# idiap/ilqr_planner

Hardware: AMD Instinct MI355X
Metric: iLQR iterations/sec (7-DoF, T=200, batch 4096) + final-cost rel-err vs Eigen ref (higher is better)
Workload: dtype f64; 1 GPU; C3: PosOrn nb_deriv=1 7-DoF Panda chain, T=200, batch 4096/GPU x 1 GPU = 4096, solver=al, 20 iterations/solve, line search on, early stop off; global_batch=4096, horizon=200, parallelism=instances sharded x1, exchange=none

## Files before the change

### ilqr_planner_amd/capi.py

```python
from __future__ import annotations

import collections
import ctypes as C
import os

import numpy as np

_HERE = os.path.dirname(os.path.abspath(__file__))
LIB_PATH = os.path.join(_HERE, "libilqr_hip.so")

MAX_SEG, MAX_KP, MAX_NX, MAX_NU, MAX_NF, MAX_NQ = 24, 8, 15, 8, 15, 13
SYS_POS_ORN, SYS_POS_ORN_TIME, SYS_JOINT, SYS_JOINT_TIME = 0, 1, 2, 3
STATUS_OK, STATUS_NONFINITE, STATUS_ALPHA_FLOOR, STATUS_SWEEP_IO = 0, 1, 2, 4
LQT_MAX_NX, LQT_MAX_NU = 16, 8
CL_STATS = 5
KP_ERR, KP_STATS, CL_OUTCOME = 5, 12, 4
CL_CON_STATS, CL_OUTCOME_CON = 6, 5
KP_ERR_POS, KP_ERR_ORN, KP_ERR_VEL, KP_ERR_ANGVEL, KP_ERR_TIME = range(5)
PROF_ROLLOUT, PROF_BACKWARD, PROF_FORWARD, PROF_OTHER, PROF_APPLY = 0, 1, 2, 3, 4
ADOPT_STATE, ADOPT_TARGETS, ADOPT_CONTROLS0, ADOPT_CONTROLS, ADOPT_MULTIPLIERS = 1, 2, 4, 8, 16
CLR_MAX_SPH, CLR_MAX_PLANES, CLR_STATS = 32, 8, 4

EXPORTS = [
    "ilqr_dims_of", "ilqr_desc_defaults", "ilqr_ctx_create", "ilqr_ctx_destroy", "ilqr_last_error", "ilqr_ctx_set_stream",
# ... 230 lines not shown
    L.ilqr_problem_closed_loop_dev.argtypes = [vp, C.c_int, vp, vp, C.c_int, vp, vp, vp]
    L.ilqr_problem_closed_loop_noise.argtypes = [vp, C.c_int, C.POINTER(Noise), dp, C.c_int, dp, dp, dp, dp, dp]
    L.ilqr_problem_closed_loop_noise_dev.argtypes = [vp, C.c_int, C.POINTER(Noise), vp, C.c_int, vp, vp, vp, vp, vp]
    L.ilqr_problem_closed_loop_report.argtypes = [vp, C.c_int, C.POINTER(Noise), dp, dp, C.c_int, C.POINTER(Tol), dp, dp, C.POINTER(Report)]
    L.ilqr_problem_closed_loop_report_dev.argtypes = [vp, C.c_int, C.POINTER(Noise), vp, vp, C.c_int, C.POINTER(Tol), vp, vp, C.POINTER(Report)]
    L.ilqr_problem_closed_loop_cov.argtypes = [vp, dp, dp, C.POINTER(Cov)]
    L.ilqr_problem_closed_loop_cov_dev.argtypes = [vp, dp, dp, C.POINTER(Cov)]
    L.ilqr_problem_closed_loop_report_con.argtypes = [vp, C.c_int, C.POINTER(Noise), dp, dp, C.c_int, C.POINTER(Tol), dp, dp, C.POINTER(Report),
                                                      C.c_double, C.POINTER(Con)]
    L.ilqr_problem_closed_loop_report_con_dev.argtypes = [vp, C.c_int, C.POINTER(Noise), vp, vp, C.c_int, C.POINTER(Tol), vp, vp, C.POINTER(Report),
                                                          C.c_double, C.POINTER(Con)]
    L.ilqr_problem_closed_loop_cov_con.argtypes = [vp, dp, dp, C.POINTER(Cov), C.POINTER(CovCon)]
    L.ilqr_problem_closed_loop_cov_con_dev.argtypes = [vp, dp, dp, C.POINTER(Cov), C.POINTER(CovCon)]
    L.ilqr_solve_recursive.argtypes = [vp, C.c_int, C.c_int, C.c_int]
    L.ilqr_solve_al.argtypes = [vp, C.c_int, C.c_int, C.c_double, C.c_double, C.c_int, C.c_int]
    L.ilqr_solve_batch_cp.argtypes = [vp, dp, C.c_int, C.c_int, C.c_int]
    L.ilqr_solve_batch.argtypes = [vp, C.c_int, C.c_int]
    for n in ("X", "fX", "U", "K", "d", "cost", "alpha", "lambda", "X_dev", "U_dev", "cost_dev"):
        getattr(L, "ilqr_problem_get_" + n).argtypes = [vp, vp]
    L.ilqr_problem_get_iters.argtypes = [vp, ip]
    L.ilqr_problem_get_status.argtypes = [vp, ip]
    L.ilqr_problem_get_trace.argtypes = [vp, dp, dp, C.c_int]
    L.ilqr_fk_batch.argtypes = [vp, C.POINTER(ProblemDesc), C.c_int, dp, dp, dp, dp]
    L.ilqr_profile_enable.argtypes = [vp, C.c_int]
    L.ilqr_profile_reset.argtypes = [vp]
    L.ilqr_profile_get.argtypes = [vp, C.c_int, dp, ip]
    L.ilqr_chain_from_urdf.argtypes = [C.c_char_p, C.c_char_p, C.c_char_p, dp, dp, C.POINTER(ProblemDesc), dp, dp]
    L.ilqr_urdf_last_error.restype = C.c_char_p
    _lib = L
    return L


def _dp(a):
    return a.ctypes.data_as(C.POINTER(C.c_double)) if a is not None else None


def _f64(x, shape=None):
    a = np.ascontiguousarray(np.asarray(x, dtype=np.float64))
    if shape is not None and tuple(a.shape) != tuple(shape):
        raise ValueError(f"expected shape {tuple(shape)}, got {a.shape}")
    return a


def _out(want, *shape):
    return np.empty(shape) if want else None


def chain_from_urdf(urdf_text: str, base: str, tip: str, tool_rpy=None, tool_xyz=None):
    L = load()
    d = ProblemDesc()
    L.ilqr_desc_defaults(C.byref(d))
    lo, up = np.zeros(MAX_SEG), np.zeros(MAX_SEG)
    rpy = _f64(tool_rpy, (3,)) if tool_rpy is not None else None
    xyz = _f64(tool_xyz, (3,)) if tool_xyz is not None else None
    if L.ilqr_chain_from_urdf(urdf_text.encode(), base.encode(), tip.encode(), _dp(rpy), _dp(xyz), C.byref(d), _dp(lo), _dp(up)):
        raise RuntimeError(L.ilqr_urdf_last_error().decode())
    n = d.n_seg
    return dict(dof=d.dof, seg_joint=[d.seg_joint[i] for i in range(n)], seg_xyz=[list(d.seg_xyz[i]) for i in range(n)],
                seg_R=[list(d.seg_R[i]) for i in range(n)], seg_axis=[list(d.seg_axis[i]) for i in range(n)],
                lower=lo[: d.dof].copy(), upper=up[: d.dof].copy())


def make_desc(*, kind, nb_deriv, horizon, dt, R_diag, chain, kp_timesteps, kp_Q, limits=None, kp_dist=None, kp_frames=None, kp_Ru=None,
              limit_multiplicity=1, kp_joint=None, limits2=None) -> ProblemDesc:
    L = load()
    d = ProblemDesc()
    L.ilqr_desc_defaults(C.byref(d))
    d.kind, d.nb_deriv, d.dof, d.horizon, d.dt = int(kind), int(nb_deriv), int(chain["dof"]), int(horizon), float(dt or 0.0)
    for i, v in enumerate(R_diag):
        d.R_diag[i] = float(v)
    n = len(chain["seg_joint"])
    if n > MAX_SEG:
        raise ValueError("too many segments")
    d.n_seg = n
    for i in range(n):
        d.seg_joint[i] = int(chain["seg_joint"][i])
        for k in range(3):
            d.seg_xyz[i][k] = float(chain["seg_xyz"][i][k])
            d.seg_axis[i][k] = float(chain["seg_axis"][i][k])
        for k in range(9):
            d.seg_R[i][k] = float(chain["seg_R"][i][k])
    dims = Dims()
    if L.ilqr_dims_of(C.byref(d), C.byref(dims)):
        raise ValueError("unsupported system kind / nb_deriv")
    if limits is not None:
        d.limits_set, d.penalty = 1, float(limits.get("penalty", 1.0))
        for i in range(len(limits["state_max"])):
            d.state_max[i] = float(limits["state_max"][i])
            d.state_min[i] = float(limits["state_min"][i])
            d.limit_weight[i] = int(limits["limit_weight"][i])
    d.n_kp = len(kp_timesteps)
    nq = dims.n_Q
    for k, (ts, Q) in enumerate(zip(kp_timesteps, kp_Q)):
        d.kp_timestep[k] = int(ts)
        jk = bool(kp_joint and kp_joint[k])
        d.kp_joint[k] = int(jk)
        nqk = dims.n_x if jk else nq
        Q = _f64(Q, (nqk, nqk))
        for a in range(nqk):
            for b in range(nqk):
                d.kp_Q[k][a * nqk + b] = Q[a, b]
    d.limit_multiplicity = int(limit_multiplicity)
    if limits2 is not None:
        d.is_sequence, d.limits2_set, d.penalty2 = 1, 1, float(limits2.get("penalty", 1.0))
        d.limit_multiplicity2 = int(limits2.get("multiplicity", 1))
        for i in range(len(limits2["state_max"])):
            d.state_max2[i] = float(limits2["state_max"][i])
            d.state_min2[i] = float(limits2["state_min"][i])
            d.limit_weight2[i] = int(limits2["limit_weight"][i])
    for k, fr in enumerate(kp_frames or []):
        if fr is not None:
            Tm = _f64(fr, (4, 4))
            d.kp_has_frame[k] = 1
            for a in range(3):
                d.kp_frame_p[k][a] = Tm[a, 3]
                for b in range(3):
                    d.kp_frame_R[k][a * 3 + b] = Tm[a, b]
    for k, ru in enumerate(kp_Ru or []):
        if ru is not None:
            d.kp_has_Ru[k] = 1
            for a, v in enumerate(ru):
                d.kp_Ru[k][a] = float(v)
    for k, kd in enumerate(kp_dist or []):
        if kd is not None:
            d.kp_dist[k] = 1
            d.kp_pos_radius[k] = float(kd["pos_radius"])
            for i in range(3):
                d.kp_orn_thresh[k][i] = float(kd["orn_thresh"][i])
    return d


class Context:
    def __init__(self, device_id: int = 0):
        import weakref

        self.L = load()
        self.h = C.c_void_p()
        self._problems = weakref.WeakSet()
        self.obstacle_path = 0
        rc = self.L.ilqr_ctx_create(device_id, C.byref(self.h))
        if rc:
            raise RuntimeError(f"ilqr_ctx_create failed (code {rc}): no usable HIP device {device_id}; there is no CPU fallback")

    def check(self, rc):
        if rc:
            raise RuntimeError(self.L.ilqr_last_error(self.h).decode())

    def set_stream(self, stream_ptr):
        self.check(self.L.ilqr_ctx_set_stream(self.h, C.c_void_p(stream_ptr)))

    def synchronize(self):
        self.check(self.L.ilqr_ctx_synchronize(self.h))

    _PINS = {"sweep": {None: 0, "mfma": 1, "rows": 2, "siwave": 4, "siwg": 5, "siwgio": 6, "siwgprep": 7}, "forward": {None: 0, "wg": 1, "dpp": 2, "wglds": 3}, "reroll": {None: 0, "rows": 1, "dpp": 2}}

    def set_crosscheck(self, generic_kernels=False, cp_lane_solve=False, cp_general=False, sweep=None, forward=None, reroll=None):
        pins = []
        for name, v in (("sweep", sweep), ("forward", forward), ("reroll", reroll)):
            if v not in self._PINS[name]:
                raise ValueError(f"set_crosscheck: {name} must be one of {[k for k in self._PINS[name] if k]} or None (got {v!r})")
            pins.append(self._PINS[name][v])
        self.check(self.L.ilqr_ctx_set_crosscheck(self.h, int(bool(generic_kernels)), int(bool(cp_lane_solve)), int(bool(cp_general)), *pins))

    def crosscheck_from_env(self):
        env = os.environ
        self.set_crosscheck(env.get("ILQR_HIP_PATH") == "v1", env.get("ILQR_CP_SOLVE") == "lane", env.get("ILQR_CP") == "general",
                            sweep=env.get("ILQR_SWEEP") or None, forward=env.get("ILQR_FWD") or None, reroll=env.get("ILQR_APPLY") or None)

    OBSTACLE_PATHS = {"generic": 0, "cooperative": 1}

    def set_obstacle_path(self, path):
        if isinstance(path, str):
            if path not in self.OBSTACLE_PATHS:
                raise ValueError(f"set_obstacle_path: path must be one of {list(self.OBSTACLE_PATHS)} (got {path!r})")
            path = self.OBSTACLE_PATHS[path]
        self.check(self.L.ilqr_ctx_set_obstacle_path(self.h, int(path)))
        self.obstacle_path = int(path)

    def set_split(self, mode: int):
        self.check(self.L.ilqr_ctx_set_split(self.h, int(mode)))

    def profile(self, on: bool):
        self.check(self.L.ilqr_profile_enable(self.h, int(on)))

    def profile_reset(self):
        self.check(self.L.ilqr_profile_reset(self.h))

    def profile_get(self, which):
        ms, n = C.c_double(), C.c_int()
        self.check(self.L.ilqr_profile_get(self.h, which, C.byref(ms), C.byref(n)))
        return ms.value, n.value

    def fk_batch(self, desc: ProblemDesc, q):
        q = _f64(q)
        n, dof = q.shape
        pos, quat, jac = np.zeros((n, 3)), np.zeros((n, 4)), np.zeros((n, 6, dof))
        self.check(self.L.ilqr_fk_batch(self.h, C.byref(desc), n, _dp(q), _dp(pos), _dp(quat), _dp(jac)))
        return pos, quat, jac

    def clearance_trajectories(self, desc: ProblemDesc, X, robot: ClrRobot, obstacles=None, traj_per_set=None, margin: float = 0.0, stats_group=None,
                               want=CLR_OUTPUTS):
        X = _f64(X)
        n, T = X.shape[0], X.shape[1]
        want = tuple(want) + (("stats",) if stats_group is not None else ())
        return _clr_host_call(lambda r, w, o: self.check(self.L.ilqr_clearance_trajectories(self.h, C.byref(desc), n, T, X.ctypes.data, r, w, o)),
                              n, T, robot, obstacles, n if traj_per_set is None else traj_per_set, margin, stats_group, want)

    def clearance_trajectories_dev(self, desc: ProblemDesc, n: int, T: int, X_ptr, robot: ClrRobot, world: ClrWorld, out: ClrOut):
        self.check(self.L.ilqr_clearance_trajectories_dev(self.h, C.byref(desc), int(n), int(T), X_ptr, C.byref(robot), C.byref(world), C.byref(out)))

    def close(self):
        if self.h:
            for p in list(self._problems):
                p.close()
            self.L.ilqr_ctx_destroy(self.h)
            self.h = C.c_void_p()

    def __del__(self):
        try:
            self.close()
        except Exception:
            pass


class BatchProblem:

    def __init__(self, ctx: Context, desc: ProblemDesc, batch: int):
        self.ctx, self.L, self.desc, self.B = ctx, ctx.L, desc, int(batch)
        self.dims = Dims()
        self.L.ilqr_dims_of(C.byref(desc), C.byref(self.dims))
        self.T, self.n_kp = desc.horizon, int(desc.n_kp)
        self.h = C.c_void_p()
        ctx.check(self.L.ilqr_problem_create(ctx.h, C.byref(desc), self.B, C.byref(self.h)))
        ctx._problems.add(self)
        self.m = 0

    def set_init_state(self, q0, dq0=None):
        q0 = _f64(q0, (self.B, self.desc.dof))
        dq0 = _f64(dq0, (self.B, self.desc.dof)) if dq0 is not None else None
        self.ctx.check(self.L.ilqr_problem_set_init_state(self.h, q0.ctypes.data, dq0.ctypes.data if dq0 is not None else None))

    def set_keypoint_targets(self, k, target):
        t = _f64(target, (self.B, self.dims.n_f))
        self.ctx.check(self.L.ilqr_problem_set_keypoint_targets(self.h, k, t.ctypes.data))

    def set_controls(self, U0):
        U0 = _f64(U0, (self.B, self.T - 1, self.dims.n_u))
        self.ctx.check(self.L.ilqr_problem_set_controls(self.h, U0.ctypes.data))

    def set_constraints(self, A, b, lambda0=None):
        A, b = _f64(A), _f64(b)
        per_step = 1 if A.ndim == 3 else 0
        self.m = A.shape[-2]
        lam = _f64(lambda0, (self.B, self.T - 1, self.m)) if lambda0 is not None else None
        self.ctx.check(self.L.ilqr_problem_set_constraints(self.h, self.m, per_step, _dp(A), _dp(b), _dp(lam)))

    def reset_multipliers(self):
        self.ctx.check(self.L.ilqr_problem_reset_multipliers(self.h))

    def set_init_state_dev(self, q0_ptr, dq0_ptr=None):
        self.ctx.check(self.L.ilqr_problem_set_init_state_dev(self.h, q0_ptr, dq0_ptr))

    def set_keypoint_targets_dev(self, k, ptr):
        self.ctx.check(self.L.ilqr_problem_set_keypoint_targets_dev(self.h, k, ptr))

    def set_controls_dev(self, ptr):
        self.ctx.check(self.L.ilqr_problem_set_controls_dev(self.h, ptr))

    def solve_recursive(self, nb_iter, line_search=True, early_stop=True):
        self.ctx.crosscheck_from_env()
        self.ctx.check(self.L.ilqr_solve_recursive(self.h, nb_iter, int(line_search), int(early_stop)))

    def solve_al(self, nb_iter, lag_update_step, penalty, scaling_factor, line_search=True, early_stop=True):
        self.ctx.crosscheck_from_env()
        self.ctx.check(self.L.ilqr_solve_al(self.h, nb_iter, lag_update_step, penalty, scaling_factor, int(line_search), int(early_stop)))

    def solve_batch_cp(self, psi, nb_iter, early_stop=True):
        psi = _f64(psi)
        assert psi.shape[0] == (self.T - 1) * self.dims.n_u
        self.ctx.crosscheck_from_env()
        self.ctx.check(self.L.ilqr_solve_batch_cp(self.h, _dp(psi), psi.shape[1], nb_iter, int(early_stop)))

    def solve_batch(self, nb_iter, early_stop=True):
        self.ctx.check(self.L.ilqr_solve_batch(self.h, nb_iter, int(early_stop)))

    def _get(self, name, shape):
        o = np.zeros(shape)
        self.ctx.check(getattr(self.L, "ilqr_problem_get_" + name)(self.h, o.ctypes.data))
        return o

    def X(self):
        return self._get("X", (self.B, self.T, self.dims.n_x))

    def fX(self):
        return self._get("fX", (self.B, self.T, self.dims.n_f))

    def U(self):
        return self._get("U", (self.B, self.T - 1, self.dims.n_u))

    def K(self):
        return self._get("K", (self.B, self.T - 1, self.dims.n_u, self.dims.n_x))

    def d(self):
        return self._get("d", (self.B, self.T - 1, self.dims.n_u))

    def cost(self):
        return self._get("cost", (self.B,))
# ... 405 lines not shown
```

### ilqr_planner_amd/csrc/ilqr_capi.cpp

```cpp
#include "../../include/ilqr_hip.h"

#include <hip/hip_runtime.h>

#include <cmath>
#include <cstdio>
#include <cstdlib>
#include <cstring>
#include <string>
#include <vector>

#include "ilqr_batchcp.hpp"
#include "ilqr_clearance.hpp"
#include "ilqr_closed_loop.hpp"
#include "ilqr_closed_loop_cov.hpp"
#include "ilqr_ctx.hpp"
#include "ilqr_kernels.hpp"
#include "ilqr_multistart.hpp"
#include "ilqr_obstacle.hpp"
#include "ilqr_plan.hpp"

using namespace ilqr;

struct DevScratch {
    double* ptr = nullptr;
    size_t elems = 0;
    int reserve(ilqr_ctx* c, size_t n) {
        if (elems >= n) return 0;
        if (ptr) { HIPCHK(c, hipStreamSynchronize(c->stream)); HIPCHK(c, hipFree(ptr)); ptr = nullptr; elems = 0; }
        HIPCHK(c, hipMalloc((void**)&ptr, n * sizeof(double)));
        elems = n;
        return 0;
    }
    void release() { if (ptr) (void)hipFree(ptr); ptr = nullptr; elems = 0; }
};

struct ilqr_problem {
    ilqr_ctx* ctx = nullptr;
    ilqr_problem_desc desc;
    ilqr_dims udims;
    ilqr_dims dims;
    DofMap map;
    bool mapped = false;
    IndexMap qmap;
    int B = 0, Bp = 0, T = 0;
    DevDesc hdesc;
    DevDesc* ddesc = nullptr;
    DevDesc* ddesc_half[2] = {nullptr, nullptr};
    int half_b0[2] = {0, 0}, half_B[2] = {0, 0};
    Bufs bufs;
    std::vector<void*> allocs;
    double *conA = nullptr, *conb = nullptr;
    double* lambda0 = nullptr;
    bool con_state_only = false;
    int trace_iters = 0;
    DevScratch staging;
    int last_nb_iter = 0;
    bool has_controls = false, has_state = false;
    bool has_gains = false;
    bool has_plan = false;
    DevScratch cl_cost;
    DevScratch cl_kpx;
    DevScratch cl_rep;
    DevScratch cl_con_ws;
    DevScratch cl_cov_ws;
    DevScratch cl_cov_kps;
    DevScratch ms_idx;
    DevScratch ms_out;
    bool has_obs = false;
    ObsArgs obs = {};
    size_t obs_sets_bytes = 0;
    ObsDense obs_dense = {};
    bool u0_zero = false;
    BatchCPState cp;
    BatchWideState cpw;
};


extern "C" const char* ilqr_version(void) { return "ilqr_hip 0.1 (gfx950, fp64)"; }

extern "C" void ilqr_desc_defaults(ilqr_problem_desc* d) {
    std::memset(d, 0, sizeof(*d));
    d->reg = 1e-6;
    d->alpha_floor = 1e-3;
    d->stop_tol = 1e-3;
    d->nb_deriv = 1;
    d->dof = 7;
}

extern "C" int ilqr_dims_of(const ilqr_problem_desc* d, ilqr_dims* o) {
    if (!d || !o) return 1;
    if (d->kind != ILQR_SYS_POS_ORN && d->kind != ILQR_SYS_POS_ORN_TIME && d->kind != ILQR_SYS_JOINT && d->kind != ILQR_SYS_JOINT_TIME) return 1;
    if (d->nb_deriv != 1 && d->nb_deriv != 2) return 1;
    if (d->kind == ILQR_SYS_JOINT || d->kind == ILQR_SYS_JOINT_TIME) {
        if (d->nb_deriv != 1) return 1;
        o->n_x = o->n_u = o->n_f = o->n_Q = d->dof + (d->kind == ILQR_SYS_JOINT_TIME ? 1 : 0);
        return 0;
    }
    const int tm = d->kind == ILQR_SYS_POS_ORN_TIME ? 1 : 0;
    o->n_x = d->nb_deriv * d->dof + tm;
    o->n_u = d->dof + tm;
    o->n_f = 7 * d->nb_deriv + tm;
    o->n_Q = o->n_f - d->nb_deriv;
    return 0;
}

extern "C" int ilqr_ctx_create(int device_id, ilqr_ctx** out) {
    if (!out) return 1;
    *out = nullptr;
    int n = 0;
    if (hipGetDeviceCount(&n) != hipSuccess || n <= 0) return 2;
    if (device_id < 0 || device_id >= n) return 3;
    if (hipSetDevice(device_id) != hipSuccess) return 4;
    auto* c = new ilqr_ctx();
    c->device = device_id;
    if (hipStreamCreateWithFlags(&c->own_stream, hipStreamNonBlocking) != hipSuccess) {
        delete c;
        return 5;
    }
    c->stream = c->own_stream;
    { int cus = 0; if (hipDeviceGetAttribute(&cus, hipDeviceAttributeMultiprocessorCount, device_id) == hipSuccess && cus > 0) c->n_simd = 4 * cus; }
    *out = c;
    return 0;
}

static void clr_release(ilqr_ctx* c);

extern "C" void ilqr_ctx_destroy(ilqr_ctx* c) {
    if (!c) return;
    (void)hipSetDevice(c->device);
    while (!c->problems.empty()) ilqr_problem_destroy(c->problems.back());
    while (!c->cleanups.empty()) { const auto cl = c->cleanups.back(); cl.destroy(cl.handle); }
    (void)hipStreamSynchronize(c->stream);
    clr_release(c);
    for (auto& p : c->pending) (void)hipEventDestroy(p.a);
    for (auto e : c->pool) (void)hipEventDestroy(e);
    for (int i = 0; i < 2; i++) {
        if (c->half_stream[i]) (void)hipStreamSynchronize(c->half_stream[i]);
        if (c->half_stream[i]) (void)hipStreamDestroy(c->half_stream[i]);
        if (c->ev_half_done[i]) (void)hipEventDestroy(c->ev_half_done[i]);
    }
    if (c->ev_begin) (void)hipEventDestroy(c->ev_begin);
    if (c->ev_stagger) (void)hipEventDestroy(c->ev_stagger);
    if (c->own_stream) (void)hipStreamDestroy(c->own_stream);
    delete c;
}

extern "C" const char* ilqr_last_error(const ilqr_ctx* c) { return c ? c->err.c_str() : "null context"; }

extern "C" int ilqr_ctx_set_stream(ilqr_ctx* c, void* s) {
    if (!c) return 1;
    c->stream = s ? (hipStream_t)s : c->own_stream;
    return 0;
}

extern "C" int ilqr_ctx_set_split(ilqr_ctx* c, int on) {
    if (!c) return 1;
    if (on < 0 || on > 2) return fail(c, "ilqr_ctx_set_split: mode must be 0, 1 or 2 (got " + std::to_string(on) + ")");
    c->split = on;
    return 0;
}

static_assert((int)SweepPin::Mfma == ILQR_XC_SWEEP_MFMA && (int)SweepPin::Rows == ILQR_XC_SWEEP_ROWS && (int)SweepPin::SiWave == ILQR_XC_SWEEP_SI_WAVE &&
              (int)SweepPin::SiWg == ILQR_XC_SWEEP_SI_WG && (int)SweepPin::SiWgIo == ILQR_XC_SWEEP_SI_WG_IO && (int)SweepPin::SiWgPrep == ILQR_XC_SWEEP_SI_WG_PREP && (int)FwdPin::Wg == ILQR_XC_FWD_WG &&
              (int)FwdPin::Dpp == ILQR_XC_FWD_DPP && (int)FwdPin::WgLds == ILQR_XC_FWD_WG_LDS && (int)RerollPin::Rows == ILQR_XC_REROLL_ROWS && (int)RerollPin::Dpp == ILQR_XC_REROLL_DPP,
              "variant pins of ilqr_plan.hpp and include/ilqr_hip.h");

extern "C" int ilqr_ctx_set_crosscheck(ilqr_ctx* c, int generic_kernels, int cp_lane_solve, int cp_general, int sweep, int forward, int reroll) {
    if (!c) return 1;
    if (sweep < 0 || sweep > 7 || sweep == 3) return fail(c, "ilqr_ctx_set_crosscheck: sweep must be ILQR_XC_AUTO, ILQR_XC_SWEEP_MFMA, ILQR_XC_SWEEP_ROWS, ILQR_XC_SWEEP_SI_WAVE, ILQR_XC_SWEEP_SI_WG, ILQR_XC_SWEEP_SI_WG_IO or ILQR_XC_SWEEP_SI_WG_PREP");
    if (forward < 0 || forward > 3) return fail(c, "ilqr_ctx_set_crosscheck: forward must be ILQR_XC_AUTO, ILQR_XC_FWD_WG, ILQR_XC_FWD_DPP or ILQR_XC_FWD_WG_LDS");
    if (reroll < 0 || reroll > 2) return fail(c, "ilqr_ctx_set_crosscheck: reroll must be ILQR_XC_AUTO, ILQR_XC_REROLL_ROWS or ILQR_XC_REROLL_DPP");
    c->xc_sweep = (SweepPin)sweep;
    c->xc_forward = (FwdPin)forward;
    c->xc_reroll = (RerollPin)reroll;
    c->xc_generic = generic_kernels != 0;
    c->xc_cp_lane = cp_lane_solve != 0;
    c->xc_cp_general = cp_general != 0;
    return 0;
}

extern "C" int ilqr_ctx_set_obstacle_path(ilqr_ctx* c, int path) {
    if (!c) return 1;
    if (path != ILQR_OBSTACLE_PATH_GENERIC && path != ILQR_OBSTACLE_PATH_COOPERATIVE)
        return fail(c, "ilqr_ctx_set_obstacle_path: path must be ILQR_OBSTACLE_PATH_GENERIC (0) or ILQR_OBSTACLE_PATH_COOPERATIVE (1) (got " + std::to_string(path) + ")");
    c->obs_coop = path == ILQR_OBSTACLE_PATH_COOPERATIVE;
    return 0;
}

extern "C" int ilqr_ctx_synchronize(ilqr_ctx* c) {
    if (!c) return 1;
    HIPCHK(c, hipStreamSynchronize(c->stream));
    return 0;
}


static hipEvent_t ev_get(ilqr_ctx* c) {
    if (!c->pool.empty()) {
        hipEvent_t e = c->pool.back();
        c->pool.pop_back();
        return e;
    }
    hipEvent_t e;
    (void)hipEventCreate(&e);
    return e;
}
static void prof_collect(ilqr_ctx* c) {
    if (c->pending.empty()) return;
    (void)hipStreamSynchronize(c->stream);
    for (size_t i = 0; i + 1 < c->pending.size(); i++) {
        const auto& p = c->pending[i];
        float ms = 0;
        if (p.which >= 0 && hipEventElapsedTime(&ms, p.a, c->pending[i + 1].a) == hipSuccess) {
            c->prof_ms[p.which] += ms;
            c->prof_n[p.which] += 1;
        }
    }
    for (auto& p : c->pending) c->pool.push_back(p.a);
    c->pending.clear();
}
static void prof_mark(ilqr_ctx* c, int which) {
    if (!c->profile) return;
    hipEvent_t e = ev_get(c);
    (void)hipEventRecord(e, c->stream);
    c->pending.push_back({e, nullptr, which});
    if (which < 0 && c->pending.size() > 4096) prof_collect(c);
}
struct ProfScope {
    ProfScope(ilqr_ctx* c, int w) { prof_mark(c, w); }
};

static void prof_hook_fn(void* c, int which) { prof_mark((ilqr_ctx*)c, which); }
static ilqr::ProfHook prof_hook(ilqr_ctx* c) {
    ilqr::ProfHook h;
    if (c->profile) { h.mark = prof_hook_fn; h.ctx = c; }
    return h;
}

extern "C" int ilqr_profile_enable(ilqr_ctx* c, int on) {
    if (!c) return 1;
    prof_collect(c);
    c->profile = on != 0;
    return 0;
}
extern "C" int ilqr_profile_reset(ilqr_ctx* c) {
    if (!c) return 1;
    prof_collect(c);
    for (int i = 0; i < ILQR_PROF_COUNT; i++) { c->prof_ms[i] = 0; c->prof_n[i] = 0; }
    return 0;
}
extern "C" int ilqr_profile_get(ilqr_ctx* c, int which, double* ms, int* n) {
    if (!c || which < 0 || which >= ILQR_PROF_COUNT) return 1;
    prof_collect(c);
    if (ms) *ms = c->prof_ms[which];
    if (n) *n = c->prof_n[which];
    return 0;
}


static void mat3(const double* A, const double* B, double* C) {
    for (int i = 0; i < 3; i++)
        for (int j = 0; j < 3; j++) C[3 * i + j] = A[3 * i] * B[j] + A[3 * i + 1] * B[3 + j] + A[3 * i + 2] * B[6 + j];
}

static_assert(DOF == DEV_DOF, "ilqr_dofmap.hpp and ilqr_device.hpp");
static_assert(STEP_MAX_KP == ILQR_MAX_KP && MAX_KP == ILQR_MAX_KP, "ilqr_steps.hpp, ilqr_device.hpp and include/ilqr_hip.h");

static int check_dof(ilqr_ctx* c, int dof) {
    if (dof < 1 || dof > DOF) return fail(c, "chains of 1 to 7 moving joints are supported (dof = " + std::to_string(dof) + ")");
    return 0;
}

static int lower_chain(ilqr_ctx* c, const ilqr_problem_desc& d, DevChain& ch) {
    if (check_dof(c, d.dof)) return 1;
    if (d.n_seg < 1 || d.n_seg > ILQR_MAX_SEG) return fail(c, "bad n_seg");
    double R[9] = {1, 0, 0, 0, 1, 0, 0, 0, 1}, p[3] = {0, 0, 0};
    int nj = 0;
    for (int s = 0; s < d.n_seg; s++) {
        double Rn[9];
        for (int i = 0; i < 3; i++) p[i] += R[3 * i] * d.seg_xyz[s][0] + R[3 * i + 1] * d.seg_xyz[s][1] + R[3 * i + 2] * d.seg_xyz[s][2];
        mat3(R, d.seg_R[s], Rn);
        std::memcpy(R, Rn, sizeof(R));
        const int j = d.seg_joint[s];
        if (j >= 0) {
            if (j != nj) return fail(c, "moving joints must be numbered 0..dof-1 in chain order");
            if (nj >= DOF) return fail(c, "chain has more than 7 moving joints (chains of 1 to 7 moving joints are supported)");
            std::memcpy(ch.Rpre[nj], R, sizeof(R));
            std::memcpy(ch.ppre[nj], p, sizeof(p));
            std::memcpy(ch.axis[nj], d.seg_axis[s], 3 * sizeof(double));
            nj++;
            const double I[9] = {1, 0, 0, 0, 1, 0, 0, 0, 1};
            std::memcpy(R, I, sizeof(R));
            p[0] = p[1] = p[2] = 0;
        }
    }
    if (nj != d.dof)
        return fail(c, "chain has " + std::to_string(nj) + " moving joints, descriptor says " + std::to_string(d.dof) + " (chains of 1 to 7 moving joints are supported)");
    for (int j = nj; j < DOF; j++) {
        const double I[9] = {1, 0, 0, 0, 1, 0, 0, 0, 1};
        std::memcpy(ch.Rpre[j], I, sizeof(I));
        for (int i = 0; i < 3; i++) ch.ppre[j][i] = ch.axis[j][i] = 0.0;
    }
    std::memcpy(ch.Rtail, R, sizeof(R));
    std::memcpy(ch.ptail, p, sizeof(p));
    return 0;
}

static int lower_desc(ilqr_ctx* c, const ilqr_problem_desc& d, const DofMap& m, int B, int Bp, DevDesc& h) {
    ilqr_dims dm;
    if (ilqr_dims_of(&d, &dm)) return fail(c, "unsupported system kind / nb_deriv");
    const IndexMap &mx = m.x, &mu = m.u;
    auto xs = [&](const double* v, int j) { return mx.usr[j] < 0 ? 0.0 : v[mx.usr[j]]; };
    auto xi = [&](const int* v, int j) { return mx.usr[j] < 0 ? 0 : v[mx.usr[j]]; };
    auto us = [&](const double* v, int j) { return v[mu.usr[j] < 0 ? 0 : mu.usr[j]]; };
    std::memset(&h, 0, sizeof(h));
    if (!((d.kind == ILQR_SYS_JOINT || d.kind == ILQR_SYS_JOINT_TIME) && d.n_seg == 0) && lower_chain(c, d, h.chain)) return 1;
    if (d.horizon < 2) return fail(c, "horizon must be >= 2");
    h.kind = d.kind; h.nd = d.nb_deriv; h.T = d.horizon; h.B = B; h.Bp = Bp; h.dt = d.dt;
    for (int j = 0; j < mu.n_dev; j++) h.R_diag[j] = us(d.R_diag, j);
    {
        const double mult = d.limit_multiplicity > 1 ? (double)d.limit_multiplicity : 1.0;
        h.limits_set = d.limits_set;
        h.penalty = d.penalty * mult;
        h.pen_xx = d.penalty * d.penalty * mult;
// ... 212 lines not shown
extern "C" int ilqr_problem_set_controls_dev(ilqr_problem* p, const double* U0) { return set_controls(p, U0, true); }

extern "C" int ilqr_problem_set_constraints(ilqr_problem* p, int m, int per_step, const double* A, const double* b, const double* lambda0) {
    if (!p) return 1;
    ilqr_ctx* c = p->ctx;
    if (m <= 0 || !A || !b) return fail(c, "bad constraint arguments");
    p->has_gains = p->has_plan = false;
    const int ns = p->dims.n_x + p->dims.n_u, T = p->T, nsu = p->udims.n_x + p->udims.n_u;
    const size_t nk = per_step ? (size_t)(T - 1) : 1;
    if (p->bufs.m != m || p->bufs.per_step != per_step || !p->conA) {
        if (p->conA) {
            HIPCHK(c, hipStreamSynchronize(c->stream));
            void* old[5] = {p->conA, p->conb, p->bufs.lambda, p->bufs.Is, p->lambda0};
            for (void* q : old) {
                for (auto it = p->allocs.begin(); it != p->allocs.end(); ++it)
                    if (*it == q) { p->allocs.erase(it); break; }
                (void)hipFree(q);
            }
            p->conA = p->conb = p->lambda0 = nullptr;
            p->bufs.lambda = p->bufs.Is = nullptr;
            p->bufs.m = 0;
        }
        if (dalloc(p, &p->conA, nk * m * ns) || dalloc(p, &p->conb, nk * m)) return 1;
        double *lam, *Is;
        if (dalloc(p, &lam, (size_t)(T - 1) * m * p->Bp) || dalloc(p, &Is, (size_t)(T - 1) * m * p->Bp)) return 1;
        p->bufs.lambda = lam;
        p->bufs.Is = Is;
        if (dalloc(p, &p->lambda0, (size_t)(T - 1) * m * p->Bp)) return 1;
    }
    std::vector<double> Aw;
    if (p->mapped) {
        const IndexMap &mx = p->map.x, &mu = p->map.u;
        Aw.assign(nk * m * ns, 0.0);
        for (size_t r = 0; r < nk * m; r++) {
            for (int j = 0; j < mx.n_user; j++) Aw[r * ns + mx.dev[j]] = A[r * nsu + j];
            for (int i = 0; i < mu.n_user; i++) Aw[r * ns + mx.n_dev + mu.dev[i]] = A[r * nsu + mx.n_user + i];
        }
    }
    HIPCHK(c, hipMemcpyAsync(p->conA, p->mapped ? Aw.data() : A, nk * m * ns * sizeof(double), hipMemcpyHostToDevice, c->stream));
    HIPCHK(c, hipMemcpyAsync(p->conb, b, nk * m * sizeof(double), hipMemcpyHostToDevice, c->stream));
    HIPCHK(c, hipStreamSynchronize(c->stream));
    p->bufs.m = m; p->bufs.per_step = per_step; p->bufs.conA = p->conA; p->bufs.conb = p->conb;
    p->con_state_only = true;
    for (size_t k = 0; k < nk * m; k++)
        for (int j = p->udims.n_x; j < nsu; j++)
            if (A[k * nsu + j] != 0.0) p->con_state_only = false;
    if (lambda0) {
        if (upload(p, lambda0, false, p->bufs.lambda, (T - 1) * m)) return 1;
    } else {
        HIPCHK(c, hipMemsetAsync(p->bufs.lambda, 0, sizeof(double) * (size_t)(T - 1) * m * p->Bp, c->stream));
    }
    HIPCHK(c, hipMemcpyAsync(p->lambda0, p->bufs.lambda, sizeof(double) * (size_t)(T - 1) * m * p->Bp, hipMemcpyDeviceToDevice, c->stream));
    return 0;
}

extern "C" int ilqr_problem_reset_multipliers(ilqr_problem* p) {
    if (!p) return 1;
    if (p->bufs.m <= 0) return fail(p->ctx, "no constraints set");
    p->has_gains = p->has_plan = false;
    HIPCHK(p->ctx, hipMemcpyAsync(p->bufs.lambda, p->lambda0, sizeof(double) * (size_t)(p->T - 1) * p->bufs.m * p->Bp,
                                  hipMemcpyDeviceToDevice, p->ctx->stream));
    return 0;
}


static int ensure_trace(ilqr_problem* p, int nb_iter) {
    if (nb_iter > p->trace_iters) {
        double *ct, *at;
        if (dalloc(p, &ct, (size_t)nb_iter * p->Bp, false) || dalloc(p, &at, (size_t)nb_iter * p->Bp, false)) return 1;
        p->bufs.cost_trace = ct;
        p->bufs.alpha_trace = at;
        p->trace_iters = nb_iter;
    }
    if (nb_iter > 0) {
        HIPCHK(p->ctx, hipMemsetAsync(p->bufs.cost_trace, 0xFF, sizeof(double) * (size_t)nb_iter * p->Bp, p->ctx->stream));
        HIPCHK(p->ctx, hipMemsetAsync(p->bufs.alpha_trace, 0xFF, sizeof(double) * (size_t)nb_iter * p->Bp, p->ctx->stream));
    }
    return 0;
}

static Bufs half_bufs(const ilqr_problem* p, int half) {
    Bufs v = p->bufs;
    const size_t o = (size_t)p->half_b0[half];
    v.desc = p->ddesc_half[half];
    for (int i = 0; i < 2; i++) { v.X[i] += o; v.U[i] += o; }
    v.U0 += o; v.q0 += o; v.dq0 += o; v.kp_tg += o;
    v.KD += o * (size_t)kd_rs(p->bufs.kd_sym, p->dims.n_u, kd_rowp(p->dims.n_x));
    v.cost += o; v.alpha += o; v.cur += o; v.active += o; v.iters += o; v.status += o; v.kpd += o; v.pend += o; v.pred += o;
    v.lsc += o; v.dun += o; v.kpdev += o; v.kpx += o; v.dunA += o;
    if (v.ws) v.ws += o;
    if (v.cost_trace) { v.cost_trace += o; v.alpha_trace += o; }
    if (v.lambda) { v.lambda += o; v.Is += o; }
    return v;
}

static PlanIn plan_input(const ilqr_problem* p, bool al, int nb_iter, int line_search) {
    const ilqr_ctx* c = p->ctx;
    const int T = p->T;
    PlanIn in;
    in.kind = p->desc.kind; in.nd = p->desc.nb_deriv; in.al = al; in.m = p->bufs.m; in.per_step = p->bufs.per_step; in.con_state_only = p->con_state_only;
    in.limits2_set = p->desc.limits2_set != 0;
    in.shared_steps = has_shared_step(p->hdesc.steps);
    in.obstacles = p->has_obs;
    in.obstacles_coop = c->obs_coop;
    in.uniform_R = true;
    for (int i = 1; i < p->dims.n_u; i++) in.uniform_R = in.uniform_R && (p->hdesc.R_diag[i] == p->hdesc.R_diag[0]);
    in.off32 = (size_t)2 * T * p->dims.n_x * p->Bp * 8 < ((size_t)1 << 32) && (size_t)T * (p->bufs.m > 0 ? p->bufs.m : 1) * p->Bp * 8 < ((size_t)1 << 32);
    in.line_search = line_search != 0; in.alpha_floor = p->desc.alpha_floor; in.nb_iter = nb_iter;
    in.B = p->B; in.n_simd = c->n_simd; in.halves = p->ddesc_half[0] != nullptr; in.split = c->split; in.profile = c->profile;
    in.generic = c->xc_generic; in.sweep = c->xc_sweep; in.forward = c->xc_forward; in.reroll = c->xc_reroll;
    return in;
}

struct Half { Bufs bufs; int B; hipStream_t st; };
static int split_begin(ilqr_problem* p, bool split, Half hv[2], int& nh) {
    ilqr_ctx* c = p->ctx;
    nh = 1;
    if (!split) {
        hv[0].bufs = p->bufs; hv[0].B = p->B; hv[0].st = c->stream;
        return 0;
    }
    for (int i = 0; i < 2; i++) {
        if (!c->half_stream[i]) HIPCHK(c, hipStreamCreateWithFlags(&c->half_stream[i], hipStreamNonBlocking));
        if (!c->ev_half_done[i]) HIPCHK(c, hipEventCreateWithFlags(&c->ev_half_done[i], hipEventDisableTiming));
    }
    if (!c->ev_begin) HIPCHK(c, hipEventCreateWithFlags(&c->ev_begin, hipEventDisableTiming));
    if (!c->ev_stagger) HIPCHK(c, hipEventCreateWithFlags(&c->ev_stagger, hipEventDisableTiming));
    HIPCHK(c, hipEventRecord(c->ev_begin, c->stream));
    nh = 2;
    for (int i = 0; i < 2; i++) {
        HIPCHK(c, hipStreamWaitEvent(c->half_stream[i], c->ev_begin, 0));
        hv[i].bufs = half_bufs(p, i); hv[i].B = p->half_B[i]; hv[i].st = c->half_stream[i];
    }
    return 0;
}
struct SplitJoin {
    ilqr_ctx* c; bool on;
    ~SplitJoin() {
        if (!on) return;
        for (int i = 0; i < 2; i++)
            if (hipEventRecord(c->ev_half_done[i], c->half_stream[i]) != hipSuccess || hipStreamWaitEvent(c->stream, c->ev_half_done[i], 0) != hipSuccess)
                (void)hipStreamSynchronize(c->half_stream[i]);
    }
};

static FwdArgs plan_fwd_args(const ilqr_problem* p, const RiccatiPlan& pl) {
    FwdArgs f;
    std::memset(&f, 0, sizeof(f));
    f.n_alpha = pl.n_alpha; f.n_kp = p->hdesc.steps.n;
    f.shared = has_shared_step(p->hdesc.steps) ? 1 : 0;
    f.n_kp_all = p->desc.n_kp;
    f.fused = pl.fused ? 1 : 0;
    f.fwd_lds = pl.fwd_lds ? 1 : 0;
    f.limits = p->desc.limits_set ? 1 : 0;
    for (int k = 0; k < p->desc.n_kp; k++) f.kp_ext |= p->desc.kp_dist[k] | p->desc.kp_has_frame[k] | p->desc.kp_has_Ru[k] | p->desc.kp_joint[k];
    return f;
}
static void launch_sweep(const ilqr_problem* p, const RiccatiPlan& pl, int h, bool al, const Bufs& bf, int B, hipStream_t st, SweepArgs& sw) {
    const int kind = p->desc.kind, nd = p->desc.nb_deriv;
    switch (pl.sweep) {
        case Sweep::SiDpp: sw.si_wg = pl.si_wg[h] ? 1 : 0; sw.si_io = pl.si_io[h] ? 1 : 0; sw.si_prep = pl.si_prep[h] ? 1 : 0; launch_backward_si_dpp(al, pl.fused, pl.kd_sym == 1, pl.si_lanes[h], bf, B, st, sw); break;
        case Sweep::Rows: launch_backward_rows(kind, nd, al, bf, B, st); break;
        case Sweep::Mfma: launch_backward_mfma(kind, nd, al, bf, B, st); break;
        case Sweep::Generic: launch_backward_generic(kind, nd, al, bf, B, st, p->has_obs ? &p->obs : nullptr); break;
    }
}
static void launch_obs_terms(const ilqr_problem* p, const RiccatiPlan& pl, const Bufs& bf, int B, hipStream_t st) {
    if (!p->has_obs) return;
    launch_obs_derivs(bf, p->obs, B, p->T, p->dims.n_x, 0, st);
    if (pl.obs_dense) launch_stage_dense(bf, p->obs, p->obs_dense.sd, B, p->T, 0, st);
}
static int ensure_obs_dense(ilqr_problem* p) {
    ilqr_ctx* c = p->ctx;
    const int N = p->dims.n_x;
    if (!p->obs_dense.sd) HIPCHK(c, hipMalloc((void**)&p->obs_dense.sd, sizeof(double) * (size_t)p->T * (size_t)(N + N * N) * (size_t)p->Bp));
    if (!p->obs_dense.part) HIPCHK(c, hipMalloc((void**)&p->obs_dense.part, sizeof(double) * (size_t)p->T * OBS_LS_ROWS * (size_t)p->Bp));
    return 0;
}

static int solve_riccati(ilqr_problem* p, bool al, int nb_iter, int lag, double penalty0, double scaling, int line_search, int early_stop) {
    if (!p) return 1;
    ilqr_ctx* c = p->ctx;
    if (!p->has_state || !p->has_controls) return fail(c, "set_init_state and set_controls must be called before a solve");
    if (nb_iter < 0) return fail(c, "nb_iter < 0");
    if (al && (p->bufs.m <= 0 || lag <= 0)) return fail(c, "AL solve needs constraints (ilqr_problem_set_constraints) and lag_update_step > 0");
    HIPCHK(c, hipSetDevice(c->device));
    if (ensure_trace(p, nb_iter)) return 1;
    p->last_nb_iter = nb_iter;
    p->has_gains = p->has_plan = false;
    const int kind = p->desc.kind, nd = p->desc.nb_deriv, T = p->T;
    const RiccatiPlan pl = plan_riccati(plan_input(p, al, nb_iter, line_search));
    if (pl.kd_sym != KD_SYM_KEEP) p->bufs.kd_sym = pl.kd_sym;
    if (pl.needs_ws && !p->bufs.ws)
        if (dalloc(p, &p->bufs.ws, (size_t)backward_ws_entries(kind, nd) * p->Bp, false)) return 1;
    if (pl.obs_dense && ensure_obs_dense(p)) return 1;

    Half hv[2];
    int nh = 1;
    if (split_begin(p, pl.split, hv, nh)) return 1;
    SplitJoin split_join{c, pl.split};
    FwdArgs f = plan_fwd_args(p, pl);
    f.line_search = line_search; f.early_stop = early_stop; f.nb_iter = nb_iter; f.penalty_roll = penalty0; f.al = al ? 1 : 0;
    if (pl.obs_dense) { f.obs = &p->obs; f.obs_part = p->obs_dense.part; f.obs_T = T; }
    for (int h = 0; h < nh; h++) {
        const Bufs& bf = hv[h].bufs;
        ProfScope ps(c, ILQR_PROF_ROLLOUT);
        if (pl.init == Init::Lti) launch_init_lti(kind, nd, bf, hv[h].B, hv[h].st);
        else launch_init(kind, nd, al, bf, hv[h].B, hv[h].st, penalty0, p->has_obs ? &p->obs : nullptr);
        if (pl.obs_dense) launch_obs_ls(bf, p->obs, p->obs_dense.part, hv[h].B, T, p->dims.n_x, 1, 1, hv[h].st);
        if (pl.init_al_update) {
            f.it = -1; f.do_update = 0;
            launch_al_update(kind, nd, bf, hv[h].B, T, hv[h].st, f);
        }
    }
    HIPCHK(c, hipGetLastError());
    double penalty = penalty0;
    SweepArgs sw;
    sw.pen_in = penalty; sw.pen_update_prev = penalty; sw.do_update_prev = 0; sw.si_wg = 0; sw.si_io = 0; sw.si_prep = 0;
    sw.sd = pl.obs_dense ? p->obs_dense.sd : nullptr;
    for (int it = 0; it < nb_iter; it++) {
        FwdArgs fi = f;
        fi.it = it;
        fi.penalty_roll = penalty;
        fi.do_update = al && ((it + 1) % lag == 0);
        if (fi.do_update) penalty *= scaling;
        fi.penalty_update = penalty;
        for (int h = 0; h < nh; h++) {
            const Bufs& bf = hv[h].bufs;
            const int B = hv[h].B;
            hipStream_t st = hv[h].st;
            if (pl.split && it == 0 && h == 1) HIPCHK(c, hipStreamWaitEvent(st, c->ev_stagger, 0));
            {
                ProfScope ps(c, ILQR_PROF_OTHER);
                launch_kp_derivs(kind, nd, bf, B, st, fi);
                launch_obs_terms(p, pl, bf, B, st);
            }
            {
                ProfScope ps(c, ILQR_PROF_BACKWARD);
                launch_sweep(p, pl, h, al, bf, B, st, sw);
            }
            if (pl.split && it == 0 && h == 0) HIPCHK(c, hipEventRecord(c->ev_stagger, st));
            {
                ProfScope ps(c, ILQR_PROF_FORWARD);
                switch (pl.forward) {
                    case Forward::WaveWg: launch_forward_wave(kind, false, bf, B, st, fi); break;
                    case Forward::WaveDpp: launch_forward_wave(kind, true, bf, B, st, fi); break;
                    case Forward::Lin: launch_forward_lin(bf, B, st, fi); break;
                    case Forward::Mfma: launch_forward_tm(kind, nd, bf, B, st, fi); break;
                    case Forward::Generic: launch_forward_generic(kind, nd, al, bf, B, st, fi, p->has_obs ? &p->obs : nullptr); break;
                }
            }
            if (pl.apply != Apply::None && (pl.apply != Apply::WaveLast || it == nb_iter - 1)) {
                ProfScope ps(c, ILQR_PROF_APPLY);
                switch (pl.apply) {
                    case Apply::Wave: case Apply::WaveLast: launch_apply_wave(kind, bf, B, T, st, fi); break;
                    case Apply::Lin: launch_apply_lin(bf, B, T, st); break;
                    case Apply::RerollRows: case Apply::RerollDpp: launch_apply_tm(kind, nd, pl.apply == Apply::RerollDpp, bf, B, st, fi); break;
                    case Apply::None: break;
                }
            }
            if (pl.al_update) {
                ProfScope ps(c, ILQR_PROF_OTHER);
                launch_al_update(kind, nd, bf, B, T, st, fi);
            }
        }
        sw.pen_in = fi.penalty_roll; sw.pen_update_prev = fi.penalty_update; sw.do_update_prev = fi.do_update;
        HIPCHK(c, hipGetLastError());
    }
    prof_mark(c, -1);
    p->has_gains = nb_iter >= 1;
    p->has_plan = true;
    return 0;
}

extern "C" int ilqr_solve_recursive(ilqr_problem* p, int nb_iter, int line_search, int early_stop) {
    return solve_riccati(p, false, nb_iter, 1, 0.0, 1.0, line_search, early_stop);
}
extern "C" int ilqr_solve_al(ilqr_problem* p, int nb_iter, int lag, double penalty, double scaling, int line_search, int early_stop) {
    return solve_riccati(p, true, nb_iter, lag, penalty, scaling, line_search, early_stop);
}

static const char* const BATCH_SHARED_STEP_TEXT =
    "keypoints that share a timestep are not supported by the batch solvers (ilqr_solve_batch_cp, ilqr_solve_batch)";
static const char* const BATCH_OBSTACLES_TEXT =
    "obstacle terms are not supported by the batch solvers (ilqr_solve_batch_cp, ilqr_solve_batch): remove them (ilqr_problem_set_obstacles with robot = NULL) or use ilqr_solve_recursive / ilqr_solve_al";

extern "C" int ilqr_solve_batch_cp(ilqr_problem* p, const double* psi, int Kw, int nb_iter, int early_stop) {
    if (!p) return 1;
    ilqr_ctx* c = p->ctx;
    if (has_shared_step(p->hdesc.steps)) return fail(c, BATCH_SHARED_STEP_TEXT);
    if (p->has_obs) return fail(c, BATCH_OBSTACLES_TEXT);
    if (!p->has_state || !p->has_controls) return fail(c, "set_init_state and set_controls must be called before a solve");
    p->has_gains = p->has_plan = false;
    HIPCHK(c, hipSetDevice(c->device));
    std::string err;
    if (ensure_trace(p, nb_iter)) return 1;
    p->last_nb_iter = nb_iter;
    const bool cp_time = p->desc.kind == ILQR_SYS_POS_ORN_TIME || p->desc.kind == ILQR_SYS_JOINT_TIME;
    std::vector<double> psiw;
    if (psi && Kw > 0 && p->mapped) {
        const IndexMap& mu = p->map.u;
        psiw.assign((size_t)(p->T - 1) * mu.n_dev * Kw, 0.0);
        for (int k = 0; k < p->T - 1; k++)
            for (int i = 0; i < mu.n_user; i++)
                std::memcpy(&psiw[((size_t)k * mu.n_dev + mu.dev[i]) * Kw], psi + ((size_t)k * mu.n_user + i) * Kw, sizeof(double) * Kw);
        psi = psiw.data();
// ... 1121 lines not shown
```

### ilqr_planner_amd/csrc/ilqr_kernels.hpp

```cpp
#pragma once
#include <hip/hip_runtime.h>

#include "ilqr_device.hpp"
#include "ilqr_dofmap.hpp"

namespace ilqr {

struct ObsArgs;

struct Bufs {
    const DevDesc* desc;
    double* X[2];
    double* U[2];
    const double* U0;
    double* KD;
    const double* q0;
    const double* dq0;
    const double* kp_tg;
    double* cost;
    double* alpha;
    int* cur;
    int* active;
    int* iters;
    int* status;
    double* kpd;
    int* pend;
    int* pred;
    double* lsc;
    double* dun;
    double* kpdev;
    double* kpx;
    double* dunA;
    double* ws;
    double* cost_trace;
    double* alpha_trace;
    int m, per_step;
    const double* conA;
    const double* conb;
    double* lambda;
    double* Is;
    int kd_sym;
};

constexpr int kd_rowp(int nx) { return (nx + 2) & ~1; }
constexpr int KD_SYM_RS = 36, KD_SYM_D = 28;
__host__ __device__ constexpr int kd_sym_tri(int i, int j) { return i * 7 - i * (i - 1) / 2 + (j - i); }
__host__ __device__ constexpr int kd_sym_off(int i, int j) { return j >= 7 ? KD_SYM_D + i : (i <= j ? kd_sym_tri(i, j) : kd_sym_tri(j, i)); }
__host__ __device__ inline int kd_off(int sym, int rowp, int i, int j) { return sym ? kd_sym_off(i, j) : i * rowp + j; }
__host__ __device__ inline int kd_rs(int sym, int nu, int rowp) { return sym ? KD_SYM_RS : nu * rowp; }
#define KD_REC(kd, Bp, RS, k, b) ((kd) + ((size_t)(k) * (size_t)(Bp) + (size_t)(b)) * (size_t)(RS))

struct FwdArgs {
    int it, line_search, early_stop, do_update, nb_iter;
    int n_kp;
    int shared;
    int n_kp_all;
    int al;
    int n_alpha;
    double penalty_roll, penalty_update;
    int kp_ext;
    int limits;
    int fused;
    int fwd_lds;
    const ObsArgs* obs;
    double* obs_part;
    int obs_T;
};

struct SweepArgs {
    double pen_in;
    double pen_update_prev;
    int do_update_prev;
    int si_wg;
    int si_io;
    int si_prep;
    const double* sd;
};

void launch_init(int kind, int nd, bool al, const Bufs& a, int B, hipStream_t st, double penalty, const ObsArgs* o = nullptr);
void launch_gains_prepare(const Bufs& a, int B, hipStream_t st);
void launch_gains_al_weights(int kind, int nd, const Bufs& a, int B, int T, double penalty, hipStream_t st);
void launch_kp_derivs(int kind, int nd, const Bufs& a, int B, hipStream_t st, const FwdArgs& f);
void launch_backward_generic(int kind, int nd, bool al, const Bufs& a, int B, hipStream_t st, const ObsArgs* o = nullptr);
int backward_ws_entries(int kind, int nd);
void launch_forward_generic(int kind, int nd, bool al, const Bufs& a, int B, hipStream_t st, const FwdArgs& f, const ObsArgs* o = nullptr);
void launch_init_lti(int kind, int nd, const Bufs& a, int B, hipStream_t st);
void launch_backward_si_dpp(bool al, bool fused, bool uniform_R, int lpi, const Bufs& a, int B, hipStream_t st, const SweepArgs& sw);
void launch_backward_rows(int kind, int nd, bool al, const Bufs& a, int B, hipStream_t st);
void launch_backward_mfma(int kind, int nd, bool al, const Bufs& a, int B, hipStream_t st);
void launch_forward_wave(int kind, bool small, const Bufs& a, int B, hipStream_t st, const FwdArgs& f);
void launch_apply_wave(int kind, const Bufs& a, int B, int T, hipStream_t st, const FwdArgs& f);
void launch_forward_lin(const Bufs& a, int B, hipStream_t st, const FwdArgs& f);
void launch_apply_lin(const Bufs& a, int B, int T, hipStream_t st);
void launch_forward_tm(int kind, int nd, const Bufs& a, int B, hipStream_t st, const FwdArgs& f);
void launch_apply_tm(int kind, int nd, bool dpp, const Bufs& a, int B, hipStream_t st, const FwdArgs& f);
void launch_al_update(int kind, int nd, const Bufs& a, int B, int T, hipStream_t st, const FwdArgs& f);
void launch_fx_all(int kind, int nd, const Bufs& a, int B, int T, double* out, hipStream_t st);
void launch_to_soa(const double* src, double* dst, int B, int Bp, int rows, hipStream_t st);
void launch_from_soa(const double* src, double* dst, int B, int Bp, int rows, hipStream_t st);
void launch_from_soa_cur(const double* s0, const double* s1, const int* cur, double* dst, int B, int Bp, int rows, hipStream_t st);
void launch_from_soa_scaled(const double* src, const double* alpha, const int* iters, double* dst, int B, int Bp, int rows, hipStream_t st);
void launch_get_gains(const double* kd, int kd_sym, const double* alpha, const int* iters, double* K_out, double* d_out, int B, int Bp, int T1, int nu, int nx, hipStream_t st);
void launch_warm_start(const Bufs& a, double* U0, double* q0, double* dq0, int shift, int B, int T, int nx, int nu, int nd, hipStream_t st);
void launch_track(const Bufs& a, const double* x_meas, int k, int with_ff, double* u_out, int B, int nx, int nu, hipStream_t st);
void launch_closed_loop_stats(const double* cost, int B, int S, double* stats, hipStream_t st);
void launch_fk_batch(const DevDesc* dd, int n, const double* q, double* pos, double* quat, double* jac, hipStream_t st);
void launch_to_soa_map(const double* src, double* dst, int B, int Bp, int outer, const IndexMap& m, hipStream_t st);
void launch_from_soa_cur_map(const double* s0, const double* s1, const int* cur, double* dst, int B, int Bp, int outer, const IndexMap& m,
                             hipStream_t st);
void launch_get_gains_map(const double* kd, int kd_sym, const double* alpha, const int* iters, double* K_out, double* d_out, int B, int Bp, int T1,
                          const DofMap& m, hipStream_t st);
void launch_track_map(const Bufs& a, const double* x_meas, int k, int with_ff, double* u_out, int B, const DofMap& m, hipStream_t st);

}
```

### ilqr_planner_amd/csrc/ilqr_kernels_dpp.hip

```cpp
#include "../../include/ilqr_hip.h"
#include "ilqr_kernels.hpp"
#include "ilqr_lanes.hpp"
#include "ilqr_step.hpp"

namespace ilqr {

namespace {

#define DPPM_ALL " row_mask:0xf bank_mask:0xf"
#define DPPM_LO " row_mask:0xf bank_mask:0x3"
#define DPPM_HI " row_mask:0xf bank_mask:0xc"


template <int LPI>
__device__ __forceinline__ void fmac_rows_all(double (&acc)[7], const double (&src)[7], const double (&mul)[7]) {
#define R_(K, LL, MASK)                                                                                                                   \
    "v_fmac_f64_dpp %[a0], %[s0], %[m" #K "] row_newbcast:" LL MASK "\n\tv_fmac_f64_dpp %[a1], %[s1], %[m" #K "] row_newbcast:" LL MASK "\n\t" \
    "v_fmac_f64_dpp %[a2], %[s2], %[m" #K "] row_newbcast:" LL MASK "\n\tv_fmac_f64_dpp %[a3], %[s3], %[m" #K "] row_newbcast:" LL MASK "\n\t" \
    "v_fmac_f64_dpp %[a4], %[s4], %[m" #K "] row_newbcast:" LL MASK "\n\tv_fmac_f64_dpp %[a5], %[s5], %[m" #K "] row_newbcast:" LL MASK "\n\t" \
    "v_fmac_f64_dpp %[a6], %[s6], %[m" #K "] row_newbcast:" LL MASK "\n\t"
#define OPS_                                                                                                                              \
    : [a0] "+v"(acc[0]), [a1] "+v"(acc[1]), [a2] "+v"(acc[2]), [a3] "+v"(acc[3]), [a4] "+v"(acc[4]), [a5] "+v"(acc[5]), [a6] "+v"(acc[6])    \
    : [s0] "v"(src[0]), [s1] "v"(src[1]), [s2] "v"(src[2]), [s3] "v"(src[3]), [s4] "v"(src[4]), [s5] "v"(src[5]), [s6] "v"(src[6]),          \
      [m0] "v"(mul[0]), [m1] "v"(mul[1]), [m2] "v"(mul[2]), [m3] "v"(mul[3]), [m4] "v"(mul[4]), [m5] "v"(mul[5]), [m6] "v"(mul[6])
    if (LPI == 16)
        asm volatile("s_nop 1\n\t" R_(0, "0", DPPM_ALL) R_(1, "1", DPPM_ALL) R_(2, "2", DPPM_ALL) R_(3, "3", DPPM_ALL) R_(4, "4", DPPM_ALL) R_(5, "5", DPPM_ALL)
                         R_(6, "6", DPPM_ALL) "s_nop 0" OPS_);
    else
        asm volatile("s_nop 1\n\t" R_(0, "0", DPPM_LO) R_(0, "8", DPPM_HI) R_(1, "1", DPPM_LO) R_(1, "9", DPPM_HI) R_(2, "2", DPPM_LO) R_(2, "10", DPPM_HI)
                         R_(3, "3", DPPM_LO) R_(3, "11", DPPM_HI) R_(4, "4", DPPM_LO) R_(4, "12", DPPM_HI) R_(5, "5", DPPM_LO) R_(5, "13", DPPM_HI)
                             R_(6, "6", DPPM_LO) R_(6, "14", DPPM_HI) "s_nop 0" OPS_);
#undef R_
#undef OPS_
}
template <int LPI>
__device__ __forceinline__ double row_dot_bc(const double (&M)[7], double src) {
    double s0, s1, s2;
#define D_(A, K, LL, MASK) "v_fmac_f64_dpp %[" A "], %[x], %[m" #K "] row_newbcast:" LL MASK "\n\t"
#define OPS_                                                                                                                       \
    : [s0] "=&v"(s0), [s1] "=&v"(s1), [s2] "=&v"(s2)                                                                                \
    : [x] "v"(src), [m0] "v"(M[0]), [m1] "v"(M[1]), [m2] "v"(M[2]), [m3] "v"(M[3]), [m4] "v"(M[4]), [m5] "v"(M[5]), [m6] "v"(M[6])
#define ZERO_ "v_mov_b64 %[s0], 0\n\tv_mov_b64 %[s1], 0\n\tv_mov_b64 %[s2], 0\n\ts_nop 1\n\t"
    if (LPI == 16)
        asm volatile(ZERO_ D_("s0", 0, "0", DPPM_ALL) D_("s1", 1, "1", DPPM_ALL) D_("s2", 2, "2", DPPM_ALL) D_("s0", 3, "3", DPPM_ALL) D_("s1", 4, "4", DPPM_ALL)
                         D_("s2", 5, "5", DPPM_ALL) D_("s0", 6, "6", DPPM_ALL) "s_nop 0" OPS_);
    else
        asm volatile(ZERO_ D_("s0", 0, "0", DPPM_LO) D_("s1", 1, "1", DPPM_LO) D_("s2", 2, "2", DPPM_LO) D_("s0", 0, "8", DPPM_HI) D_("s1", 1, "9", DPPM_HI)
                         D_("s2", 2, "10", DPPM_HI) D_("s0", 3, "3", DPPM_LO) D_("s1", 4, "4", DPPM_LO) D_("s2", 5, "5", DPPM_LO) D_("s0", 3, "11", DPPM_HI)
                             D_("s1", 4, "12", DPPM_HI) D_("s2", 5, "13", DPPM_HI) D_("s0", 6, "6", DPPM_LO) "s_nop 1\n\t" D_("s0", 6, "14", DPPM_HI) "s_nop 0" OPS_);
#undef D_
#undef OPS_
#undef ZERO_
    return (s0 + s1) + s2;
}

#define PV_HEAD16_(C) "v_mov_b64_dpp %[acc], %[s" #C "] row_newbcast:" #C DPPM_ALL "\n\t"
#define PV_HEAD8_(C, C8) "v_mov_b64_dpp %[acc], %[s" #C "] row_newbcast:" #C DPPM_LO "\n\tv_mov_b64_dpp %[acc], %[s" #C "] row_newbcast:" #C8 DPPM_HI "\n\t"
#define PV_RCP_(C)                                                                                                                \
    "v_rcp_f64 %[rc], %[acc]\n\t"                                                                                                 \
    "v_fma_f64 %[t], %[s" #C "], %[n" #C "], %[s" #C "]\n\t"                                                                      \
    "v_fma_f64 %[e], -%[acc], %[rc], 1.0\n\t"                                                                                     \
    "v_fma_f64 %[e], %[e], %[e], %[e]\n\t"                                                                                        \
    "v_fma_f64 %[rc], %[e], %[rc], %[rc]\n\t"                                                                                     \
    "v_mul_f64 %[t], %[t], %[rc]\n\t"
#define PV_F_(J, LL, MASK) "v_fmac_f64_dpp %[s" #J "], %[s" #J "], -%[t] row_newbcast:" LL MASK "\n\t"
#define PV_TAIL_(C) "v_add_f64 %[s" #C "], %[t], %[n" #C "]\n\tv_fma_f64 %[myrc], -%[rc], %[n" #C "], %[myrc]\n\t"
#define PV16_(C, A, B, D, E, F, G) PV_HEAD16_(C) PV_RCP_(C) PV_F_(A, #C, DPPM_ALL) PV_F_(B, #C, DPPM_ALL) PV_F_(D, #C, DPPM_ALL) PV_F_(E, #C, DPPM_ALL) PV_F_(F, #C, DPPM_ALL) PV_F_(G, #C, DPPM_ALL) PV_TAIL_(C)
#define PV8_(C, C8, A, B, D, E, F, G)                                                                                              \
    PV_HEAD8_(C, C8) PV_RCP_(C) PV_F_(A, #C, DPPM_LO) PV_F_(B, #C, DPPM_LO) PV_F_(D, #C, DPPM_LO) PV_F_(E, #C, DPPM_LO) PV_F_(F, #C, DPPM_LO) PV_F_(G, #C, DPPM_LO) \
        PV_F_(A, #C8, DPPM_HI) PV_F_(B, #C8, DPPM_HI) PV_F_(D, #C8, DPPM_HI) PV_F_(E, #C8, DPPM_HI) PV_F_(F, #C8, DPPM_HI) PV_F_(G, #C8, DPPM_HI) PV_TAIL_(C)
template <int LPI>
__device__ __forceinline__ void pivots(double (&s)[7], const double (&nm1)[7], double& myrc) {
    double acc, rc, e, t;
#define OPS_                                                                                                                              \
    : [acc] "=&v"(acc), [rc] "=&v"(rc), [e] "=&v"(e), [t] "=&v"(t), [s0] "+v"(s[0]), [s1] "+v"(s[1]), [s2] "+v"(s[2]), [s3] "+v"(s[3]),     \
      [s4] "+v"(s[4]), [s5] "+v"(s[5]), [s6] "+v"(s[6]), [myrc] "+v"(myrc)                                                                  \
    : [n0] "v"(nm1[0]), [n1] "v"(nm1[1]), [n2] "v"(nm1[2]), [n3] "v"(nm1[3]), [n4] "v"(nm1[4]), [n5] "v"(nm1[5]), [n6] "v"(nm1[6])
    if (LPI == 16)
        asm volatile("s_nop 1\n\t" PV16_(0, 1, 2, 3, 4, 5, 6) PV16_(1, 0, 2, 3, 4, 5, 6) PV16_(2, 0, 1, 3, 4, 5, 6) PV16_(3, 0, 1, 2, 4, 5, 6) PV16_(4, 0, 1, 2, 3, 5, 6)
                         PV16_(5, 0, 1, 2, 3, 4, 6) PV16_(6, 0, 1, 2, 3, 4, 5) "s_nop 0" OPS_);
    else
        asm volatile("s_nop 1\n\t" PV8_(0, 8, 1, 2, 3, 4, 5, 6) PV8_(1, 9, 0, 2, 3, 4, 5, 6) PV8_(2, 10, 0, 1, 3, 4, 5, 6) PV8_(3, 11, 0, 1, 2, 4, 5, 6)
                         PV8_(4, 12, 0, 1, 2, 3, 5, 6) PV8_(5, 13, 0, 1, 2, 3, 4, 6) PV8_(6, 14, 0, 1, 2, 3, 4, 5) "s_nop 0" OPS_);
#undef OPS_
}

__device__ __forceinline__ double oct_row_g(double a_l, double x_l, double b) {
#pragma clang fp contract(off)
    const double p = a_l * x_l;
    return oct_sum_rounded(p) - b;
}

__device__ __forceinline__ unsigned lds_addr(const void* p) { return (unsigned)(size_t)(const __attribute__((address_space(3))) void*)p; }
typedef __attribute__((address_space(3))) int lds_int;
__device__ __forceinline__ int flag_read(const int* p) { LDS_ORDER(); const int v = *(const lds_int*)p; LDS_ORDER(); return v; }
__device__ __forceinline__ void flag_write(int* p, int v) { LDS_ORDER(); *(lds_int*)p = v; LDS_ORDER(); }
__device__ __forceinline__ int wait_consumed(int seen, unsigned addr, int need);
__device__ __forceinline__ double ldg(const double* base, unsigned byte_off) { return *reinterpret_cast<const double*>(reinterpret_cast<const char*>(base) + byte_off); }
__device__ __forceinline__ void stg(double* base, unsigned byte_off, double v) { *reinterpret_cast<double*>(reinterpret_cast<char*>(base) + byte_off) = v; }

}

constexpr int SW_WAVES = 4;
constexpr int SW_RING = 8;
constexpr int SW_POLL_CHAIN = 1 << 20;
constexpr int SW_POLL_IO = 1 << 18;
constexpr int SW_PREP = 2;
constexpr int SW_PRING = 8;
constexpr int SW_PENT = 6;
namespace {
__device__ __forceinline__ int wait_consumed(int seen, unsigned addr, int need) {
    int v = seen, cons, cnt;
    asm volatile(
        "s_mov_b32 %[cnt], 0\n"
        "1:\n\t"
        "v_readfirstlane_b32 %[cons], %[v]\n\t"
        "s_cmp_ge_i32 %[cons], %[need]\n\t"
        "s_cbranch_scc1 2f\n\t"
        "s_cmp_ge_u32 %[cnt], %[lim]\n\t"
        "s_cbranch_scc1 2f\n\t"
        "s_sleep 1\n\t"
        "ds_read_b32 %[v], %[addr]\n\t"
        "s_add_u32 %[cnt], %[cnt], 1\n\t"
        "s_waitcnt lgkmcnt(0)\n\t"
        "s_branch 1b\n"
        "2:"
        : [v] "+v"(v), [cons] "=&s"(cons), [cnt] "=&s"(cnt)
        : [addr] "v"(addr), [need] "s"(need), [lim] "s"(SW_POLL_CHAIN)
        : "memory", "scc");
    return __builtin_amdgcn_readfirstlane(cons < need ? 1 : 0);
}
}
template <int LPI, int MR, bool FUSED, bool UNIF, bool WG = false, int IO = 0>
__global__ __launch_bounds__(WG ? (SW_WAVES + ((IO & 7) ? 1 : 0) + ((IO & 4) ? SW_PREP : 0)) * 64 : 64) void k_backward_si_dpp(Bufs a, SweepArgs sw) {
    constexpr int IOW = IO & 7;
    constexpr bool DENSE = (IO & 8) != 0;
    constexpr int N = 7, IPW = 64 / LPI;
    static_assert(!DENSE || (!FUSED && !WG && IOW == 0), "the dense form: lone waves, the accepted trajectory in memory");
    constexpr int NWV = WG ? SW_WAVES : 1;
    constexpr bool IOK = (IOW & 1) != 0, IOX = (IOW & 2) != 0;
    constexpr bool PRP = (IOW & 4) != 0;
    constexpr int NIMG = IOK ? SW_RING : 2, XRING = SW_RING, XROW = 18;
    static_assert(!PRP || (IOK && IOX && FUSED && SW_PRING == XRING && SW_WAVES * (64 / LPI) == 8 * SW_PREP), "the preparing waves: on top of the full I/O wave, one x | u slot per prepared slot");
    static_assert(!WG || (LPI == 16 && FUSED), "the workgroup form: 4 instances per wave, 16 per workgroup = one 128-byte line per row segment");
    static_assert(!IOW || (WG && MR <= 1), "the I/O wave: workgroup form, at most one constraint row (256 VGPRs at two waves on a SIMD)");
    constexpr int MRR = MR > 0 ? MR : 1;
    constexpr int ROWP = kd_rowp(N), RS = UNIF ? KD_SYM_RS : N * ROWP;
    static_assert(ROWP == 8, "a gain row is the lane's eight doubles {K_r0..K_r6, d_r}");
    static_assert(LPI == 8 || LPI == 16, "");
    constexpr int NPQ_ = (IPW * (RS / 2) + 63) / 64, IMG = (IPW * RS > 128 * NPQ_) ? IPW * RS : 128 * NPQ_;
    __shared__ __attribute__((aligned(16))) double sKw[NWV][NIMG][IMG + 64];
    __shared__ double sXU[IOX ? XRING : 1][IOX ? 2 * N + 1 : 1][IOX ? XROW : 1];
    __shared__ __attribute__((aligned(16))) double sPr[PRP ? SW_PRING : 1][PRP ? 8 * SW_WAVES * (64 / LPI) : 1][PRP ? SW_PENT : 2];
    __shared__ int sFl[IOW ? NWV + 1 + (PRP ? SW_PREP : 0) : 1];
    const DevDesc& d = *a.desc;
    const int wv = WG ? __builtin_amdgcn_readfirstlane((int)threadIdx.x >> 6) : 0;
    double (*const sK)[IMG + 64] = sKw[wv < NWV ? wv : 0];
    const int lane = WG ? (int)threadIdx.x & 63 : (int)threadIdx.x, g = lane / LPI, l = lane % LPI;
    const int r = l & 7;
    const bool low = l < 8;
    const int b0 = (xcd_tile() * NWV + wv) * IPW;
    const int b = b0 + g;
    const int Bp = d.Bp, T = d.T;
    const bool ok = (b < d.B) && a.active[b < d.B ? b : 0];
    const int bb = (b < d.B) ? b : 0;
    const int pendw = (FUSED && b < d.B) ? a.pend[bb] : 0;
    const bool acc = pendw > 0;
    if (IOW) {
        constexpr int RS_ = UNIF ? KD_SYM_RS : N * kd_rowp(N), PCS_ = RS_ / 2, NPQ2 = (IPW * PCS_ + 63) / 64;
        if (wv == NWV) {
            const int bi = xcd_tile() * (NWV * IPW) + (lane & 15);
            const bool in = bi < d.B;
            const int bbi = in ? bi : 0;
            const bool oki = in && a.active[bbi];
            const int pwi = in ? a.pend[bbi] : 0;
            const int curi = a.cur[bbi];
            __syncthreads();
            const unsigned okm16 = (unsigned)__ballot((oki && lane < 16) ? 1 : 0);
            const unsigned livem = (unsigned)__ballot(((oki || pwi > 0) && lane < 16) ? 1 : 0);
            if (livem == 0u) return;
            bool live[NWV], kfull[NWV], pst[NWV][NPQ2];
            UNR for (int w = 0; w < NWV; w++) {
                live[w] = ((livem >> (w * IPW)) & 15u) != 0u;
                kfull[w] = ((okm16 >> (w * IPW)) & 15u) == 15u;
                UNR for (int q = 0; q < NPQ2; q++) {
                    const int c = lane + 64 * q, gi = (c / PCS_ < IPW) ? c / PCS_ : 0;
                    pst[w][q] = c < IPW * PCS_ && ((okm16 >> (w * IPW + gi)) & 1u);
                }
            }
            const bool want = (lane < NWV) ? ((livem >> (lane * IPW)) & 15u) != 0u : false;
            const int T1 = d.T - 1, Bpi = d.Bp;
            double* Ko = KD_REC(a.KD, Bpi, RS_, T1 - 1, xcd_tile() * (NWV * IPW));
            const ptrdiff_t Ks = (ptrdiff_t)Bpi * RS_;
            const bool blendi = pwi > 1;
            const unsigned bufoi = (unsigned)((a.X[1] - a.X[0]) * (ptrdiff_t)sizeof(double));
            const unsigned Vs = (unsigned)N * Bpi * 8u;
            unsigned oXi = (unsigned)(1 - curi) * bufoi + ((unsigned)((T1 - 1) * N) * Bpi + bbi) * 8u;
            for (int n = 1; n <= T1; n++) {
                for (int spins = 0;; spins++) {
                    const int pv = flag_read(&sFl[lane < NWV ? lane : 0]);
                    if (__ballot((want && pv < n) ? 1 : 0) == 0ull) break;
                    if (spins >= SW_POLL_IO) {
                        if (lane < 16 && in) { a.active[bbi] = 0; atomicOr(&a.status[bbi], ILQR_STATUS_SWEEP_IO); }
                        return;
                    }
                    __builtin_amdgcn_s_sleep(4);
                }
                LDS_ORDER();
                double kqa[NWV][NPQ2], kqb[NWV][NPQ2], xu[4];
                if (IOK) {
                    UNR for (int w = 0; w < NWV; w++) UNR for (int q = 0; q < NPQ2; q++) {
                        const double2 t2 = reinterpret_cast<const double2*>(sKw[w][(n - 1) % SW_RING])[lane + 64 * q];
                        kqa[w][q] = t2.x; kqb[w][q] = t2.y;
                    }
                }
                if (IOX) { UNR for (int q = 0; q < 4; q++) xu[q] = sXU[(n - 1) % XRING][(4 * q + (lane >> 4)) < 2 * N ? 4 * q + (lane >> 4) : 2 * N][lane & 15]; }
                flag_write(&sFl[NWV], n);
                if (IOK) {
                    UNR for (int w = 0; w < NWV; w++) {
                        if (!live[w]) continue;
                        double2* dst = reinterpret_cast<double2*>(Ko + w * (IPW * RS_)) + lane;
                        if (kfull[w]) {
                            UNR for (int q = 0; q + 1 < NPQ2; q++) dst[64 * q] = make_double2(kqa[w][q], kqb[w][q]);
                            if (lane + 64 * (NPQ2 - 1) < IPW * PCS_) dst[64 * (NPQ2 - 1)] = make_double2(kqa[w][NPQ2 - 1], kqb[w][NPQ2 - 1]);
                        } else {
                            UNR for (int q = 0; q < NPQ2; q++) if (pst[w][q]) dst[64 * q] = make_double2(kqa[w][q], kqb[w][q]);
                        }
                    }
                    Ko -= Ks;
                }
                if (IOX) {
                    if (blendi) {
                        UNR for (int q = 0; q < 4; q++) {
                            const int row = 4 * q + (lane >> 4);
                            if (row < N) stg(a.X[0], oXi + (unsigned)row * Bpi * 8u, xu[q]);
                            else if (row < 2 * N) stg(a.U[0], oXi + (unsigned)(row - N) * Bpi * 8u, xu[q]);
                        }
                    }
                    oXi -= Vs;
                }
            }
            return;
        }
        if (PRP && wv > NWV) {
            const int pw = wv - NWV - 1, iw = pw * 8 + (lane >> 3), rp = lane & 7;
            const int bi = xcd_tile() * (NWV * IPW) + iw;
            const bool in = bi < d.B;
            const int bbi = in ? bi : 0;
            const bool oki = in && a.active[bbi];
            const int pwi = in ? a.pend[bbi] : 0;
            const int curi = a.cur[bbi];
            __syncthreads();
            if (__ballot((oki || pwi > 0) ? 1 : 0) == 0ull) return;
            const bool acci = pwi > 0, blendi = pwi > 1;
            const double aacc = acci ? ldexp(1.0, -(pwi - 1)) : 1.0;
            int rd = curi, r1 = blendi ? 1 - curi : curi;
            if (acci && !blendi) rd = r1 = 1 - curi;
            const bool updi = acci && sw.do_update_prev;
            const bool isVp = rp < N;
            const int vp = isVp ? rp : 0;
            const int Bpp = d.Bp, Tp = d.T;
            const int lim_on = d.limits_set;
            const double pen = d.penalty, pen_xx = d.pen_xx;
            const int lw_v = isVp ? d.lw[vp] : 0;
            const double smax_v = lw_v != 0 ? d.smax[vp] : __builtin_inf(), smin_v = lw_v != 0 ? d.smin[vp] : -__builtin_inf();
            const double Avp = (MR == 1 && isVp) ? a.conA[vp] : 0.0, bp = (MR == 1) ? a.conb[0] : 0.0;
            double* const Xb = a.X[0];
            double* const Ub = a.U[0];
            const unsigned bufo = (unsigned)((a.X[1] - a.X[0]) * (ptrdiff_t)sizeof(double));
            const unsigned Vstep = (unsigned)N * Bpp * 8u, Lstep = (unsigned)MR * Bpp * 8u;
            unsigned oA = (unsigned)rd * bufo + ((unsigned)((Tp - 2) * N + vp) * Bpp + bbi) * 8u;
            unsigned oB = (unsigned)r1 * bufo + ((unsigned)((Tp - 2) * N + vp) * Bpp + bbi) * 8u;
            unsigned oL = ((unsigned)(Tp - 2) * MR * Bpp + bbi) * 8u, oLw = oL;
            constexpr int PF = 4;
            double xr[PF], ur[PF], x1r[PF], u1r[PF], lr[PF];
            auto fetch = [&](int slot, int kk) {
                xr[slot] = ldg(Xb, oA);
                ur[slot] = ldg(Ub, oA);
                x1r[slot] = ldg(Xb, oB);
                u1r[slot] = ldg(Ub, oB);
                lr[slot] = 0;
                if (MR > 0) lr[slot] = ldg(a.lambda, oL);
                if (kk > 0) { oA -= Vstep; oB -= Vstep; oL -= Lstep; }
            };
// ... 400 lines not shown
```

### ilqr_planner_amd/csrc/ilqr_kernels_wave.hip

```cpp
#include <cstdlib>
#include <cstring>

#include "ilqr_lanes.hpp"
#include "ilqr_obstacle.hpp"
#include "ilqr_plan.hpp"
#include "ilqr_step.hpp"

namespace ilqr {

#ifndef FW_IW
#define FW_IW 16
#endif
template <int NA>
__global__ __launch_bounds__(FW_IW * 32) void k_forward_wg(Bufs a, FwdArgs f) {
    constexpr int NX = 7, NU = 7, ROWP = kd_rowp(NX), RS = NU * ROWP, NR = NX + NU;
    static_assert(ROWP == 8, "record row = 7 gains + feed-forward");
    constexpr int S = 8, PF = S - 1;
    constexpr int IW = FW_IW, NT = IW * 32;
    constexpr int NSEG = S * NR;
    constexpr int NRND = (NSEG * IW + NT - 1) / NT;
    __shared__ double sIn[2][NSEG][IW];
    __shared__ double sOut[NSEG][IW];

    const DevDesc& d = *a.desc;
    const int tid = threadIdx.x, wv = tid >> 6, lane = tid & 63, g = lane >> 5, r8 = (lane >> 2) & 7, jl = lane & 3;
    const int b0 = xcd_tile() * IW;
    const int Bp = d.Bp, T = d.T, B = d.B;
    {
        const int bi = b0 + (lane & (IW - 1));
        const bool any = (bi < B) && (a.active[bi < B ? bi : 0] != 0);
        if (__ballot(any ? 1 : 0) == 0ull) return;
    }
    const int li = wv * 2 + g;
    const int b = b0 + li;
    const bool inst_ok = (b < B) && (a.active[b < B ? b : 0] != 0);
    const int bb = (b < B) ? b : 0;
    const int r = r8 < NU ? r8 : NU - 1;
    const int c0 = 2 * jl, c1 = 2 * jl + 1;
    const bool c1ok = c1 < NX;
    const int c1c = c1ok ? c1 : NX - 1;
    const bool colst = inst_ok && (r8 == 0);
    const bool rowst = inst_ok && (jl == 0) && (r8 < NU);
    const int src0 = (g * 32 + c0 * 4) * 4, src1 = (g * 32 + c1c * 4) * 4;

    const double dt = d.dt, dt1 = c1ok ? dt : 0.0;
    const int lim_on = d.limits_set;
    const double pen = d.penalty;
    const int lw0 = d.lw[c0], lw1 = c1ok ? d.lw[c1c] : 0;
    const double mx0 = lw0 ? d.smax[c0] : INFINITY, mn0 = lw0 ? d.smin[c0] : -INFINITY;
    const double mx1 = lw1 ? d.smax[c1c] : INFINITY, mn1 = lw1 ? d.smin[c1c] : -INFINITY;
    const int n_kp = d.n_kp;
    int kpi = 0, kp_next = (n_kp > 0) ? d.kp_t[0] : -1;

    const int l_inst = tid % IW;
    const int l_b = (b0 + l_inst < B) ? b0 + l_inst : 0;
    const bool l_ok = (b0 + l_inst < B) && (a.active[l_b] != 0);
    const int l_cur = a.cur[l_b];
    const double* l_src[NRND];
    double* l_dst[NRND];
    int l_s[NRND], l_kmax[NRND];
    size_t l_stride[NRND];
    bool l_valid[NRND];
    UNR for (int q = 0; q < NRND; q++) {
        const int seg = (q * NT + tid) / IW;
        l_valid[q] = seg < NSEG;
        const int sg = l_valid[q] ? seg : 0;
        const int s = sg / NR, row = sg % NR;
        l_s[q] = s;
        if (row < NX) {
            l_src[q] = a.X[l_cur] + (size_t)row * Bp + l_b;
            l_dst[q] = a.X[1 - l_cur] + (size_t)row * Bp + l_b;
            l_stride[q] = (size_t)NX * Bp;
            l_kmax[q] = T - 1;
        } else {
            l_src[q] = a.U[l_cur] + (size_t)(row - NX) * Bp + l_b;
            l_dst[q] = a.U[1 - l_cur] + (size_t)(row - NX) * Bp + l_b;
            l_stride[q] = (size_t)NU * Bp;
            l_kmax[q] = T - 2;
        }
    }
    double pre[NRND];
    auto block_load = [&](int k0) {
        UNR for (int q = 0; q < NRND; q++) {
            const int k = k0 + l_s[q];
            pre[q] = l_src[q][(size_t)(k < l_kmax[q] ? k : l_kmax[q]) * l_stride[q]];
        }
    };
    auto block_stage = [&](int buf) {
        UNR for (int q = 0; q < NRND; q++)
            if (l_valid[q]) (&sIn[buf][0][0])[q * NT + tid] = pre[q];
    };
    auto block_store = [&](int k0) {
        UNR for (int q = 0; q < NRND; q++) {
            const int k = k0 + l_s[q];
            if (l_valid[q] && l_ok && k <= l_kmax[q]) l_dst[q][(size_t)k * l_stride[q]] = (&sOut[0][0])[q * NT + tid];
        }
    };

    const int sym = a.kd_sym, rs_ = kd_rs(sym, NU, ROWP);
    const double* pK = a.KD + (size_t)bb * rs_ + kd_off(sym, ROWP, r, c0);
    const double* pK1 = a.KD + (size_t)bb * rs_ + kd_off(sym, ROWP, r, c1);
    const size_t sK_ = (size_t)Bp * rs_;
    double rk0[S], rk1[S];
    auto fetch = [&](int slot, int k) {
        if (sym) {
            rk0[slot] = *pK;
            rk1[slot] = *pK1;
        } else {
            const double2 v2 = *reinterpret_cast<const double2*>(pK);
            rk0[slot] = v2.x;
            rk1[slot] = v2.y;
        }
        if (k < T - 2) { pK += sK_; pK1 += sK_; }
    };
    block_load(0);
    __builtin_amdgcn_sched_barrier(0);
    UNR for (int q = 0; q < PF; q++) { fetch(q, q); __builtin_amdgcn_sched_barrier(0); }
    block_stage(0);
    block_load(S);
    lds_barrier();

    double dx0 = 0, dx1 = c1ok ? 0.0 : 1.0, dun = 0, pcA = 0, pcB = 0;

    auto seg_bad = [&](double xa, double xb) -> bool {
        const double ea = xa + dx0, eb = xb + dx1;
        return (fmax(xa, ea) > mx0) | (fmin(xa, ea) < mn0) | (fmax(xb, eb) > mx1) | (fmin(xb, eb) < mn1);
    };
    auto limit_cost_of = [&](double v, double mx, double mn) -> double {
        const double q = fmax(v - mx, 0.0) + fmax(mn - v, 0.0);
        return q * pen * q;
    };
    const double myA = ldexp(1.0, -r8), myB = ldexp(1.0, -(r8 + 8));
    auto limits_all = [&](double xb0, double xb1) {
        pcA += limit_cost_of(fma(myA, dx0, xb0), mx0, mn0) + limit_cost_of(fma(myA, dx1, xb1), mx1, mn1);
        if (NA > 8) pcB += limit_cost_of(fma(myB, dx0, xb0), mx0, mn0) + limit_cost_of(fma(myB, dx1, xb1), mx1, mn1);
    };
    double* kpdev = a.kpdev;

    const int nblocks = (T + S - 1) / S;
    for (int j = 0; j < nblocks; j++) {
        const int k0 = j * S, buf = j & 1;
        UNR for (int s = 0; s < S; s++) {
            const int k = k0 + s;
            fetch((s + PF) % S, k + PF);
            if (k > T - 1) continue;
            const double xb0 = sIn[buf][s * NR + c0][li], xb1 = sIn[buf][s * NR + c1c][li];
            if (k < T - 1) {
                const double ub = sIn[buf][s * NR + NX + r][li];
                const double du = quad_sum(fma(rk0[s], dx0, rk1[s] * dx1));
                const double du0 = bperm_f64(src0, du), du1 = bperm_f64(src1, du);
                if (colst) {
                    sOut[s * NR + c0][li] = xb0 + dx0;
                    if (c1ok) sOut[s * NR + c1][li] = xb1 + dx1;
                }
                if (rowst) sOut[s * NR + NX + r][li] = ub + du;
// ... 24 lines not shown
                    double* o = kpdev + (size_t)kpi * NR * Bp;
                    AT(o, c0, bb) = dx0;
                    if (c1ok) AT(o, c1, bb) = dx1;
                }
            }
        }
        lds_barrier();
        block_store(k0);
        block_stage(buf ^ 1);
        block_load(k0 + 2 * S);
        lds_barrier();
    }
    {
        const double sA = quad_sum(pcA), sB = quad_sum(pcB);
        if (inst_ok && jl == 0) {
            if (r8 < NA) AT(a.lsc, r8, bb) = sA;
            if (NA > 8 && r8 + 8 < NA) AT(a.lsc, r8 + 8, bb) = sB;
        }
    }
    if (colst && jl == 0) a.dun[bb] = dun;
}


#define FD_LO " row_mask:0xf bank_mask:0x3"
#define FD_HI " row_mask:0xf bank_mask:0xc"
__device__ __forceinline__ double fd_half_dot(const double (&K)[4], double x, double one) {
    double s0, s1, s2;
#define D_(A, J, C, M, X) "v_fmac_f64_dpp %[" A "], %[" X "], %[k" #J "] row_newbcast:" #C M "\n\t"
    asm volatile("v_mov_b64 %[s0], 0\n\tv_mov_b64 %[s1], 0\n\tv_mov_b64 %[s2], 0\n\ts_nop 1\n\t"
                 D_("s0", 0, 0, FD_LO, "x") D_("s1", 1, 1, FD_LO, "x") D_("s2", 2, 2, FD_LO, "x") D_("s0", 0, 4, FD_HI, "x") D_("s1", 1, 5, FD_HI, "x") D_("s2", 2, 6, FD_HI, "x")
                 D_("s0", 3, 3, FD_LO, "x") D_("s1", 3, 0, FD_HI, "one") "s_nop 0"
                 : [s0] "=&v"(s0), [s1] "=&v"(s1), [s2] "=&v"(s2)
                 : [x] "v"(x), [one] "v"(one), [k0] "v"(K[0]), [k1] "v"(K[1]), [k2] "v"(K[2]), [k3] "v"(K[3]));
#undef D_
    return (s0 + s1) + s2;
}

template <int NA, bool LIM, bool ES>
__device__ __forceinline__ bool forward_dpp_body(const Bufs& a, const FwdArgs& f) {
    constexpr int NX = 7, NU = 7, ROWP = kd_rowp(NX), RS = NU * ROWP, PF = 8;
    static_assert(ROWP == 8, "record row = 7 gains + feed-forward");
    const DevDesc& d = *a.desc;
    const int lane = threadIdx.x, g = lane >> 4, l = lane & 15, h = l >> 3, r8 = l & 7;
    const int b = xcd_tile() * 4 + g;
    const int Bp = d.Bp, T = d.T, B = d.B;
    const bool inst_ok = (b < B) && (a.active[b < B ? b : 0] != 0);
    if (__ballot(inst_ok ? 1 : 0) == 0ull) return false;
    const int bb = (b < B) ? b : 0;
    const bool row = r8 < NX;
    const int r = row ? r8 : NX - 1;
    const bool st = inst_ok && row;
    const bool sx = st && h == 0;
    const int cur = a.cur[bb];
    const double dt = d.dt, pen = d.penalty, one = 1.0;
    const int lw = LIM ? d.lw[r] : 0;
    const double mx = lw ? d.smax[r] : INFINITY, mn = lw ? d.smin[r] : -INFINITY;
    const int n_kp = d.n_kp;
    int kpi = 0, kp_next = (n_kp > 0) ? d.kp_t[0] : -1;

    const size_t Vstep = (size_t)NX * Bp;
    const double* pV = (h ? a.U[cur] : a.X[cur]) + (size_t)r * Bp + bb;
    const int sym = a.kd_sym, rs_ = kd_rs(sym, NU, ROWP);
    const double* kb = a.KD;
    unsigned ko[4];
    UNR for (int j = 0; j < 4; j++) ko[j] = ((unsigned)bb * rs_ + (sym ? kd_sym_off(r, 4 * h + j) : r * ROWP + 4 * h + j)) * 8u;
    const size_t Kstep = (size_t)Bp * rs_;
    double* qV = (h ? a.U[1 - cur] : a.X[1 - cur]) + (size_t)r * Bp + bb;
    const double xT = a.X[cur][((size_t)(T - 1) * NX + r) * Bp + bb];

    double Kr[PF][4], vr[PF];
    auto fetch = [&](int slot, int kk) {
        const char* kbb = reinterpret_cast<const char*>(kb);
        if (sym) {
            UNR for (int j = 0; j < 4; j++) Kr[slot][j] = *reinterpret_cast<const double*>(kbb + ko[j]);
        } else {
            const double2 v0 = *reinterpret_cast<const double2*>(kbb + ko[0]), v1 = *reinterpret_cast<const double2*>(kbb + ko[2]);
            Kr[slot][0] = v0.x; Kr[slot][1] = v0.y; Kr[slot][2] = v1.x; Kr[slot][3] = v1.y;
        }
        vr[slot] = *pV;
        const bool more = kk < T - 2;
        kb += more ? Kstep : 0; pV += more ? Vstep : 0;
    };
    UNR for (int q = 0; q < PF; q++) { fetch(q, q); __builtin_amdgcn_sched_barrier(0); }

    double dx = 0, dun = 0, pc[NA];
    UNR for (int i = 0; i < NA; i++) pc[i] = 0;
    auto limit_cost_of = [&](double v) -> double {
        const double q = fmax(v - mx, 0.0) + fmax(mn - v, 0.0);
        return q * pen * q;
    };
    auto limits_all = [&](double xb) {
        UNR for (int i = 0; i < NA; i++) pc[i] += limit_cost_of(fma(ldexp(1.0, -i), dx, xb));
    };
    auto seg_bad = [&](double xb) -> bool {
        const double e = xb + dx;
        return (fmax(xb, e) > mx) | (fmin(xb, e) < mn);
    };
    double* kpdev = a.kpdev;

#define FD_STEP_(JJ, CHK)                                                                                          \
    {                                                                                                              \
        const int k = k0 + JJ;                                                                                     \
        if (!CHK || k < T - 1) {                                                                                   \
            const double vb = vr[JJ];                                                         \
            const double part = fd_half_dot(Kr[JJ], dx, one);                                                      \
            const double du = part + dpp_f64<0x128>(part);                   \
            if (st) *qV = vb + (h ? du : dx);                                                                      \
            qV += Vstep;                                                                                           \
            if (ES) dun += __builtin_amdgcn_sqrt(oct_sum(row ? du * du : 0.0));                \
            if (LIM && __builtin_expect(__ballot((seg_bad(vb) & sx) ? 1 : 0) != 0ull, 0)) limits_all(vb);          \
            if (CHK && k == kp_next) {                            \
                double* o = kpdev + (size_t)kpi * (NX + NU) * Bp;                                                  \
                if (st) AT(o, h * NX + r, bb) = h ? du : dx;                                                       \
                kpi++;                                                                                             \
                kp_next = (kpi < n_kp) ? __builtin_amdgcn_readfirstlane(d.kp_t[kpi]) : -1;                         \
            }                                                                                                      \
            dx = dx + dt * du;                                               \
        }                                                                                                          \
        __builtin_amdgcn_sched_barrier(0);                           \
        fetch(JJ, k + PF);                                                                                         \
    }
    for (int k0 = 0; k0 < T - 1; k0 += PF) {
        const bool plain = (k0 + PF <= T - 1) && (kp_next < 0 || kp_next >= k0 + PF);
        if (plain) {
            FD_STEP_(0, false) FD_STEP_(1, false) FD_STEP_(2, false) FD_STEP_(3, false) FD_STEP_(4, false) FD_STEP_(5, false) FD_STEP_(6, false) FD_STEP_(7, false)
        } else {
            FD_STEP_(0, true) FD_STEP_(1, true) FD_STEP_(2, true) FD_STEP_(3, true) FD_STEP_(4, true) FD_STEP_(5, true) FD_STEP_(6, true) FD_STEP_(7, true)
        }
    }
#undef FD_STEP_
    static_assert(PF == 8, "eight step copies above");
    {
        if (sx) *qV = xT + dx;
        if (LIM && __ballot((seg_bad(xT) & sx) ? 1 : 0) != 0ull) limits_all(xT);
        if (kp_next == T - 1 && sx) {
            double* o = kpdev + (size_t)kpi * (NX + NU) * Bp;
            AT(o, r, bb) = dx;
        }
    }
    UNR for (int i = 0; i < NA; i++) {
        const double sA = LIM ? oct_sum(row ? pc[i] : 0.0) : 0.0;
        if (inst_ok && l == 0) AT(a.lsc, i, bb) = sA;
    }
    if (inst_ok && l == 0) a.dun[bb] = dun;
    return true;
}
template <int NA, bool LIM, bool ES>
__global__ __launch_bounds__(64) void k_forward_dpp(Bufs a, FwdArgs f) { (void)forward_dpp_body<NA, LIM, ES>(a, f); }
#undef FD_LO
#undef FD_HI

constexpr int FR_WAVES = 4;
constexpr int FR_PF = 8;
template <bool LIM, bool ES, bool SYM>
__global__ __launch_bounds__(FR_WAVES * 64) void k_forward_reg(Bufs a, FwdArgs f) {
#pragma clang fp contract(off)
    constexpr int NX = 7, NU = 7, ROWP = kd_rowp(NX), PF = FR_PF, IPW = 4;
    static_assert(ROWP == 8, "record row = 7 gains + feed-forward");
    static_assert(PF >= 2 && PF % 2 == 0, "image parity = slot parity");
    constexpr int RSD = SYM ? KD_SYM_RS : NU * ROWP;
    constexpr int NPC = IPW * RSD / 2;
    static_assert(NPC > 64 && NPC <= 128, "two pieces per lane");
    __shared__ __attribute__((aligned(16))) double sK[FR_WAVES][2][IPW * RSD];
    constexpr int NR = NX + NU, IWG = FR_WAVES * IPW, OSTR = IWG + 2, NT = FR_WAVES * 64, NOUT = PF * NR * IWG, NRND = (NOUT + NT - 1) / NT;
    __shared__ double sOut[2][PF * NR * OSTR];
    const DevDesc& d = *a.desc;
    const int wv = __builtin_amdgcn_readfirstlane((int)threadIdx.x >> 6);
    const int lane = threadIdx.x & 63, g = lane >> 4, l = lane & 15, h = l >> 3, r8 = l & 7;
    const int b0 = (xcd_tile() * FR_WAVES + wv) * IPW;
    const int b = b0 + g;
    const int Bp = d.Bp, T = d.T, B = d.B;
    const bool inst_ok = (b < B) && (a.active[b < B ? b : 0] != 0);
    {
        const int bi = b0 - wv * IPW + (lane & (IWG - 1));
        const bool any = (bi < B) && (a.active[bi < B ? bi : 0] != 0);
        if (__ballot(any ? 1 : 0) == 0ull) return;
    }
    const int bb = (b < B) ? b : 0;
    const bool row = r8 < NX;
    const int r = row ? r8 : NX - 1;
    const bool st = inst_ok && row;
    const bool sx = st && h == 0;
    const int cur = a.cur[bb];
    const double dt = d.dt, pen = d.penalty;
    const int lw = LIM ? d.lw[r] : 0;
    const double mx = lw ? d.smax[r] : INFINITY, mn = lw ? d.smin[r] : -INFINITY;
    const int n_kp = d.n_kp;
    int kpi = 0, kp_next = (n_kp > 0) ? d.kp_t[0] : -1;

    const size_t Vstep = (size_t)NX * Bp;
    const double* pV = (h ? a.U[cur] : a.X[cur]) + (size_t)r * Bp + bb;
    static_assert(IWG == 16, "a row segment of the workgroup's instances is one 128-byte line");
    const int tid = wv * 64 + lane, l_inst = tid & (IWG - 1), l_bi = b0 - wv * IPW + l_inst, l_b = l_bi < B ? l_bi : 0;
    const bool l_ok = (l_bi < B) && (a.active[l_b] != 0);
    double* l_dst[NRND];
    int l_s[NRND], l_src[NRND];
    {
        const int l_cur = a.cur[l_b];
        UNR for (int q = 0; q < NRND; q++) {
            const int e = q * NT + tid, seg = (e < NOUT ? e : 0) / IWG, s_ = seg / NR, rw = seg % NR;
            l_s[q] = e < NOUT ? s_ : PF;
            l_src[q] = seg * OSTR + l_inst;
            l_dst[q] = (rw < NX ? a.X[1 - l_cur] + (size_t)rw * Bp : a.U[1 - l_cur] + (size_t)(rw - NX) * Bp) + (size_t)s_ * Vstep + l_b;
        }
    }
    const int ow = (h * NX + r) * OSTR + wv * IPW + g;
    auto block_store = [&](int buf, int k0) {
        UNR for (int q = 0; q < NRND; q++) {
            const double v = sOut[buf][l_src[q]];
            if (l_ok && l_s[q] < PF && k0 + l_s[q] < T - 1) l_dst[q][(size_t)k0 * Vstep] = v;
        }
    };
    const double xT = a.X[cur][((size_t)(T - 1) * NX + r) * Bp + bb];
    const char* kb = reinterpret_cast<const char*>(a.KD + (size_t)b0 * RSD);
    const size_t Kstep = (size_t)Bp * RSD * sizeof(double);
    const int p1 = (64 + lane < NPC) ? 64 + lane : lane;
    const unsigned ko0 = lane * 16u, ko1 = p1 * 16u;
    double* const img = &sK[wv][0][0];
    constexpr int IMG = IPW * RSD;
    int ro[4];
    UNR for (int j = 0; j < 4; j++) ro[j] = g * RSD + (SYM ? kd_sym_off(r, 4 * h + j) : r * ROWP + 4 * h + j);

    double ga[PF], gb[PF], gc[PF], gd[PF], vr[PF];
    auto fetch_g = [&](int slot, int kk) {
        typedef double d2v __attribute__((ext_vector_type(2)));
        const d2v v0 = __builtin_nontemporal_load(reinterpret_cast<const d2v*>(kb + ko0)), v1 = __builtin_nontemporal_load(reinterpret_cast<const d2v*>(kb + ko1));
        ga[slot] = v0.x; gb[slot] = v0.y; gc[slot] = v1.x; gd[slot] = v1.y;
        kb += (kk < T - 2) ? Kstep : 0;
    };
    auto fetch_v = [&](int slot, int kk) {
        vr[slot] = *pV;
        pV += (kk < T - 2) ? Vstep : 0;
    };
    auto stage = [&](int slot, int buf) {
        const double ta = ring_take(ga[slot]), tb = ring_take(gb[slot]), tc = ring_take(gc[slot]), td = ring_take(gd[slot]);
        *reinterpret_cast<double2*>(img + buf * IMG + 2 * lane) = make_double2(ta, tb);
        *reinterpret_cast<double2*>(img + buf * IMG + 2 * p1) = make_double2(tc, td);
    };
    auto pick = [&](int buf, double (&K)[4]) {
        if (SYM) {
            UNR for (int j = 0; j < 4; j++) K[j] = img[buf * IMG + ro[j]];
        } else {
            const double2 v0 = *reinterpret_cast<const double2*>(img + buf * IMG + ro[0]), v1 = *reinterpret_cast<const double2*>(img + buf * IMG + ro[2]);
            K[0] = v0.x; K[1] = v0.y; K[2] = v1.x; K[3] = v1.y;
        }
    };
    UNR for (int q = 0; q < PF; q++) { fetch_g(q, q); fetch_v(q, q); __builtin_amdgcn_sched_barrier(0); }
    double Kc[4];
    stage(0, 0);
    LDS_ORDER();
    pick(0, Kc);
    stage(1, 1);
    LDS_ORDER();
    __builtin_amdgcn_sched_barrier(0);
    fetch_g(0, PF);
    fetch_g(1, PF + 1);

    double dx = 0, dun = 0, pc[4] = {0, 0, 0, 0};
    auto pair_cost = [&](double v0, double mx0, double mn0, double v1, double mx1, double mn1) -> double {
        const double q0 = fmax(v0 - mx0, 0.0) + fmax(mn0 - v0, 0.0), q1 = fmax(v1 - mx1, 0.0) + fmax(mn1 - v1, 0.0);
        return fma(q0 * pen, q0, (q1 * pen) * q1);
    };
    const double myA = ldexp(1.0, -l);
    double pmx[8], pmn[8];
    UNR for (int c = 0; c < 8; c++) {
        const int lwc = (LIM && c < NX) ? d.lw[c < NX ? c : 0] : 0;
        pmx[c] = lwc ? d.smax[c < NX ? c : 0] : INFINITY;
        pmn[c] = lwc ? d.smin[c < NX ? c : 0] : -INFINITY;
    }
#define FR_PAIR_(J, C1, DX1)                                                                                                        \
    pc[J] += pair_cost(fma(myA, dppz_bcast<2 * J>(dx), dppz_bcast<2 * J>(xb)), pmx[2 * J], pmn[2 * J],                              \
                       fma(myA, DX1, dppz_bcast<C1>(xb)), pmx[2 * J + 1], pmn[2 * J + 1]);
    auto limits_all = [&](double xb) {
        FR_PAIR_(0, 1, dppz_bcast<1>(dx)) FR_PAIR_(1, 3, dppz_bcast<3>(dx)) FR_PAIR_(2, 5, dppz_bcast<5>(dx)) FR_PAIR_(3, 6, 1.0)
    };
    auto seg_bad = [&](double xb) -> bool {
        const double e = xb + dx;
        return (fmax(xb, e) > mx) | (fmin(xb, e) < mn);
    };
    const bool ev = (r8 & 1) == 0, last2 = r8 >= 6;
    double* kpdev = a.kpdev;

#define FR_STEP_(JJ, CHK)                                                                                          \
    {                                                                                                              \
        const int k = k0 + JJ;                                                                                     \
        double Kn[4];                                                                                              \
        pick((JJ + 1) & 1, Kn);                                                     \
        LDS_ORDER();                                                                                               \
        stage((JJ + 2) % PF, JJ & 1);                                     \
        LDS_ORDER();                                                                                               \
        __builtin_amdgcn_sched_barrier(0);                           \
        fetch_g((JJ + 2) % PF, k + 2 + PF);                                                                        \
        if (!CHK || k < T - 1) {                                                                                   \
            const double vb = ring_take(vr[JJ]);                                              \
            const double x0 = dpp_bcast_halves<0, 4>(dx), x1 = dpp_bcast_halves<1, 5>(dx);                         \
            const double x2 = dpp_bcast_halves<2, 6>(dx), x3 = dpp_bcast_halves<3, -1>(dx, 1.0);                   \
            const double part = fma(Kc[0], x0, Kc[1] * x1) + fma(Kc[2], x2, Kc[3] * x3);                           \
            const double du = part + dpp_f64<0x128>(part);                   \
            sOut[ob][JJ * NR * OSTR + ow] = vb + (h ? du : dx);                               \
            if (ES) {                                     \
                const double o = dpp_f64<0xB1>(du);                                      \
                const double pa = ev ? du : o, pb = ev ? o : du;                                                   \
                double s = fma(pa, pa, last2 ? 0.0 : pb * pb);                                                     \
                s = s + dpp_f64<0x4E>(s);                                            \
                s = s + dpp_f64<0x141>(s);                                                                         \
                dun += __builtin_amdgcn_sqrt(s);                                                                   \
            }                                                                                                      \
            if (LIM && __builtin_expect(__ballot((seg_bad(vb) & sx) ? 1 : 0) != 0ull, 0)) limits_all(vb);          \
            if (CHK && k == kp_next) {                            \
                double* o = kpdev + (size_t)kpi * (NX + NU) * Bp;                                                  \
                if (st) AT(o, h * NX + r, bb) = h ? du : dx;                                                       \
                kpi++;                                                                                             \
                kp_next = (kpi < n_kp) ? __builtin_amdgcn_readfirstlane(d.kp_t[kpi]) : -1;                         \
            }                                                                                                      \
            dx = fma(dt, du, dx);                                            \
        }                                                                                                          \
        __builtin_amdgcn_sched_barrier(0);                                                                         \
        fetch_v(JJ, k + PF);                                                                                       \
        UNR for (int j = 0; j < 4; j++) Kc[j] = Kn[j];                                                             \
    }
    for (int k0 = 0, ob = 0; k0 < T - 1; k0 += PF, ob ^= 1) {
        UNR for (int jj = 0; jj < PF; jj++) FR_STEP_(jj, true)
        lds_barrier();
        block_store(ob, k0);
    }
#undef FR_STEP_
    {
        if (sx) a.X[1 - cur][((size_t)(T - 1) * NX + r) * Bp + bb] = xT + dx;
        if (LIM && __ballot((seg_bad(xT) & sx) ? 1 : 0) != 0ull) limits_all(xT);
        if (kp_next == T - 1 && sx) {
            double* o = kpdev + (size_t)kpi * (NX + NU) * Bp;
            AT(o, r, bb) = dx;
        }
    }
#undef FR_PAIR_
    const double sA = LIM ? (pc[0] + pc[1]) + (pc[2] + pc[3]) : 0.0;
    const int na = f.n_alpha <= 1 ? 1 : f.n_alpha <= 11 ? 11 : 16;
    if (inst_ok && l < na) AT(a.lsc, l, bb) = sA;
    if (inst_ok && l == 0) a.dun[bb] = dun;
}

template <int NA>
__device__ __forceinline__ int select_decide(const Bufs& a, const FwdArgs& f, const DevDesc& d, int bb, bool inst_ok, bool mine, int gi, int al, int n_alpha, double c,
                                             bool* stopped = nullptr) {
    const int Bp = d.Bp;
    if (mine) c += AT(a.lsc, al, bb);
    const double cost0 = a.cost[bb];
    const bool okc = mine && !((c >= cost0) || isnan(c));
    const unsigned m16 = (unsigned)((__ballot(okc ? 1 : 0) >> (gi * 16)) & 0xffffull);
    const int w = m16 ? (__ffs(m16) - 1) : (n_alpha - 1);
    const double wcost = __shfl(c, gi * 16 + w);
    bool stop = false;
    if (inst_ok && al == 0) {
        const double walpha = ldexp(1.0, -w);
        a.cost[bb] = wcost;
        a.alpha[bb] = walpha;
        a.iters[bb] = f.it + 1;
        a.status[bb] = (isfinite(wcost) ? 0 : 1) | ((walpha <= d.alpha_floor) ? 2 : 0);
        if (a.cost_trace) {
            a.cost_trace[(size_t)f.it * Bp + bb] = wcost;
            a.alpha_trace[(size_t)f.it * Bp + bb] = walpha;
        }
        a.pend[bb] = w + 1;
        a.pred[bb] = w;
        stop = f.early_stop && (walpha * sqrt(walpha * a.dun[bb]) < d.stop_tol);
        if (!f.al) stop = stop && (wcost < 1e-3);
        if (stop) a.active[bb] = 0;
    }
    if (stopped) *stopped = __shfl(stop ? 1 : 0, gi * 16) != 0;
    return w;
}

template <class S, int NA, bool EXT, int KW>
__global__ __launch_bounds__(64 * KW) void k_select(Bufs a, FwdArgs f) {
    constexpr int NX = S::NX, NU = S::NU;
    static_assert(NA <= 16, "16 lanes per instance");
    static_assert(KW == 1 || KW == 2, "one or two waves per four instances");
    __shared__ double sc[KW == 2 ? MAX_KP : 1][64];
    const DevDesc& d = *a.desc;
    const int lane = threadIdx.x & 63, wv = threadIdx.x >> 6, gi = lane >> 4, al = lane & 15;
    const int b = blockIdx.x * 4 + gi;
    const int Bp = d.Bp, T = d.T, B = d.B;
    const bool inst_ok = (b < B) && (a.active[b < B ? b : 0] != 0);
    const int bb = (b < B) ? b : 0;
    const int n_alpha = f.n_alpha < NA ? f.n_alpha : NA;
    const bool mine = inst_ok && al < n_alpha;
    const double aa = ldexp(1.0, -al);
    double c = 0;
    if (mine) {
        const double* Xb = a.X[a.cur[bb]];
        const double* Ub = a.U[a.cur[bb]];
        for (int kpi = wv; kpi < d.n_kp; kpi += KW) {
            const int k = d.kp_t[kpi];
            const double* dv = a.kpdev + (size_t)kpi * (NX + NU) * Bp;
            double xt[NX], ut[NU], tg[S::NF];
            UNR for (int i = 0; i < NX; i++) xt[i] = fma(aa, AT(dv, i, bb), AT(Xb, k * NX + i, bb));
            UNR for (int i = 0; i < NU; i++) ut[i] = (k < T - 1) ? fma(aa, AT(dv, NX + i, bb), AT(Ub, k * NU + i, bb)) : 0.0;
            UNR for (int i = 0; i < S::NF; i++) tg[i] = AT(a.kp_tg, kpi * S::NF + i, bb);
            const double ck = kp_cost<S, EXT>(d, kpi, tg, xt, ut);
            if (KW == 1) c += ck;
            else sc[kpi][lane] = ck;
        }
    }
    if (KW == 2) {
        __syncthreads();
        if (wv != 0) return;
        if (mine) { for (int kpi = 0; kpi < d.n_kp; kpi++) c += sc[kpi][lane]; }
    }
    (void)select_decide<NA>(a, f, d, bb, inst_ok, mine, gi, al, n_alpha, c);
}

template <class S>
__device__ __forceinline__ double con_g_oct(const Bufs& a, int r, const double* x) {
#pragma clang fp contract(off)
    static_assert(S::NX == 7, "the register-resident sweep: single-integrator systems of seven joints");
    const double* Ar = a.conA + (size_t)r * (S::NX + S::NU);
    double p[8];
    UNR for (int j = 0; j < 7; j++) p[j] = Ar[j] * x[j];
    p[7] = 0.0 * x[0];
    const double q0 = (p[0] + p[1]) + (p[2] + p[3]);
    const double q1 = (p[4] + p[5]) + (p[6] + p[7]);
    return (q0 + q1) - a.conb[r];
}

template <class S>
__global__ __launch_bounds__(256) void k_apply(Bufs a, FwdArgs f) {
    constexpr int NX = S::NX, NU = S::NU;
    const DevDesc& d = *a.desc;
    const int tid = threadIdx.x, inst = tid & 15, hi = tid >> 4;
    const int b = blockIdx.x * 16 + inst, k = blockIdx.y * 16 + hi;
    const int Bp = d.Bp, T = d.T;
    if (b >= d.B || k >= T) return;
    const int w = a.pend[b] - 1;
    if (w < 0) return;
    const int cur = a.cur[b];
    const double aa = ldexp(1.0, -w);
    const double* Xb = a.X[cur];
    const double* Ub = a.U[cur];
    double* Xn = a.X[1 - cur];
    double* Un = a.U[1 - cur];
    const int m = f.al ? a.m : 0;
    if (w == 0 && (m == 0 || k == T - 1)) return;
    double x[NX], u[NU];
    UNR for (int i = 0; i < NX; i++) x[i] = AT(Xn, k * NX + i, b);
    if (k < T - 1) { UNR for (int i = 0; i < NU; i++) u[i] = AT(Un, k * NU + i, b); }
    if (w > 0) {
        double xb[NX], ub[NU];
        UNR for (int i = 0; i < NX; i++) xb[i] = AT(Xb, k * NX + i, b);
        if (k < T - 1) { UNR for (int i = 0; i < NU; i++) ub[i] = AT(Ub, k * NU + i, b); }
        UNR for (int i = 0; i < NX; i++) {
            x[i] = fma(aa, x[i] - xb[i], xb[i]);
            AT(Xn, k * NX + i, b) = x[i];
        }
        if (k < T - 1) {
            UNR for (int i = 0; i < NU; i++) {
                u[i] = fma(aa, u[i] - ub[i], ub[i]);
                AT(Un, k * NU + i, b) = u[i];
            }
        }
    }
    if (k < T - 1) {
        for (int r = 0; r < m; r++) {
            const double g = f.fused ? con_g_oct<S>(a, r, x) : con_g<S>(a, k, r, x, u);
            const double lam = AT(a.lambda, k * m + r, b);
            AT(a.Is, k * m + r, b) = f.penalty_roll * ((g < 0 && lam == 0) ? 0.0 : 1.0);
            if (f.do_update) {
                const double v = f.fused ? fma(f.penalty_update, g, lam) : lam + f.penalty_update * g;
                AT(a.lambda, k * m + r, b) = v > 0 ? v : 0;
            }
        }
    }
}
template <class S>
__global__ __launch_bounds__(256) void k_al_post(Bufs a, FwdArgs f) {
    const DevDesc& d = *a.desc;
    const int b = blockIdx.x * 256 + threadIdx.x;
    const int k = blockIdx.y;
    if (b >= d.B) return;
    if (a.iters[b] != f.it + 1) return;
    const int Bp = d.Bp;
    const int cur = a.cur[b];
    double x[S::NX], u[S::NU];
    UNR for (int i = 0; i < S::NX; i++) x[i] = AT(a.X[cur], k * S::NX + i, b);
    UNR for (int i = 0; i < S::NU; i++) u[i] = AT(a.U[cur], k * S::NU + i, b);
    for (int r = 0; r < a.m; r++) {
        const double g = con_g<S>(a, k, r, x, u);
        const double lam = AT(a.lambda, k * a.m + r, b);
        AT(a.Is, k * a.m + r, b) = f.penalty_roll * ((g < 0 && lam == 0) ? 0.0 : 1.0);
        if (f.do_update) {
            const double v = lam + f.penalty_update * g;
            AT(a.lambda, k * a.m + r, b) = v > 0 ? v : 0;
        }
    }
}
__global__ void k_flip_ran(Bufs a) {
    const int b = blockIdx.x * blockDim.x + threadIdx.x;
    if (b >= a.desc->B) return;
    if (a.pend[b] > 0) {
        a.cur[b] = 1 - a.cur[b];
        a.pend[b] = 0;
    }
}

template <class S>
__global__ __launch_bounds__(256) void k_init_roll_lti(Bufs a) {
    constexpr int NX = S::NX, NU = S::NU, ND = S::ND, TM = S::TM, CH = 8;
    const DevDesc& d = *a.desc;
    const int b = blockIdx.x * 256 + threadIdx.x, i = blockIdx.y;
    if (b >= d.B) return;
    const int Bp = d.Bp, T = d.T;
    const bool isT = TM && i == DOF;
    const int ij = isT ? 0 : i;
    const int xrow = isT ? NX - 1 : i, urow = isT ? NU - 1 : i;
    const double pen = d.penalty;
    const bool lim = d.limits_set != 0 && !isT;
    const double mxq = (lim && d.lw[ij]) ? d.smax[ij] : INFINITY, mnq = (lim && d.lw[ij]) ? d.smin[ij] : -INFINITY;
    const double mxv = (lim && ND == 2 && d.lw[DOF + ij]) ? d.smax[DOF + ij] : INFINITY, mnv = (lim && ND == 2 && d.lw[DOF + ij]) ? d.smin[DOF + ij] : -INFINITY;
    auto lcost = [&](double v, double mx, double mn) { const double q = fmax(v - mx, 0.0) + fmax(mn - v, 0.0); return q * pen * q; };
    double q = isT ? 0.0 : AT(a.q0, ij, b), v = (ND == 2 && !isT) ? AT(a.dq0, ij, b) : 0.0, cost = 0;
    const double* __restrict__ U0 = a.U0;
    double* __restrict__ X = a.X[0];
    double* __restrict__ U = a.U[0];
    for (int k0 = 0; k0 < T - 1; k0 += CH) {
        double u[CH], us[CH];
        UNR for (int j = 0; j < CH; j++) {
            const int kk = (k0 + j < T - 1 ? k0 + j : T - 2);
            u[j] = AT(U0, kk * NU + urow, b);
            us[j] = TM ? AT(U0, kk * NU + NU - 1, b) : 0.0;
        }
        UNR for (int j = 0; j < CH; j++) {
            const int k = k0 + j;
            if (k >= T - 1) break;
            const double dt = TM ? us[j] * us[j] : d.dt;
            AT(X, k * NX + xrow, b) = q;
            if (ND == 2 && !isT) AT(X, k * NX + DOF + ij, b) = v;
            AT(U, k * NU + urow, b) = u[j];
            cost += lcost(q, mxq, mnq);
            if (ND == 2) cost += lcost(v, mxv, mnv);
            if (isT) {
                q = q + dt;
            } else if (ND == 1) {
                q = q + (dt * u[j] + dt * dt / 2 * 0.0);
            } else {
                q = q + (dt * v + dt * dt / 2 * u[j]);
                v = v + dt * u[j];
            }
        }
    }
    AT(X, (T - 1) * NX + xrow, b) = q;
    if (ND == 2 && !isT) AT(X, (T - 1) * NX + DOF + ij, b) = v;
    cost += lcost(q, mxq, mnq);
    if (ND == 2) cost += lcost(v, mxv, mnv);
    if (!isT) AT(a.lsc, ij, b) = cost;
}

template <class S>
__global__ __launch_bounds__(64) void k_init_finish(Bufs a) {
    constexpr int NX = S::NX, NU = S::NU;
    const DevDesc& d = *a.desc;
    const int b = blockIdx.x * 64 + threadIdx.x;
    if (b >= d.B) return;
    const int Bp = d.Bp, T = d.T;
    double cost = 0;
    for (int kpi = 0; kpi < d.n_kp; kpi++) {
        const int k = d.kp_t[kpi];
        double x[NX], u[NU], tg[S::NF];
        UNR for (int i = 0; i < NX; i++) x[i] = AT(a.X[0], k * NX + i, b);
        UNR for (int i = 0; i < NU; i++) u[i] = (k < T - 1) ? AT(a.U[0], k * NU + i, b) : 0.0;
        UNR for (int i = 0; i < S::NF; i++) tg[i] = AT(a.kp_tg, kpi * S::NF + i, b);
        cost += kp_cost<S>(d, kpi, tg, x, u);
    }
    if (d.limits_set) { UNR for (int i = 0; i < DOF; i++) cost += AT(a.lsc, i, b); }
    a.cost[b] = cost;
    a.alpha[b] = 1.0;
    a.cur[b] = 0;
    a.active[b] = 1;
    a.iters[b] = 0;
    a.pend[b] = 0;
    a.pred[b] = 0;
    a.status[b] = isfinite(cost) ? 0 : 1;
}

static_assert(SysAll::same_as<SysAll>([](int kind, int nd) { return init_lti_supported(kind, nd); }), "k_init_roll_lti: every system");
void launch_init_lti(int kind, int nd, const Bufs& a, int B, hipStream_t st) {
    SysAll::dispatch(kind, nd, [&](auto s) {
        using S = decltype(s);
        hipLaunchKernelGGL((k_init_roll_lti<S>), dim3((B + 255) / 256, DOF + S::TM), dim3(256), 0, st, a);
        hipLaunchKernelGGL((k_init_finish<S>), dim3((B + 63) / 64), dim3(64), 0, st, a);
    });
}
void launch_al_update(int kind, int nd, const Bufs& a, int B, int T, hipStream_t st, const FwdArgs& f) {
    SysAll::dispatch(kind, nd, [&](auto s) {
        hipLaunchKernelGGL((k_al_post<decltype(s)>), dim3((B + 255) / 256, T - 1), dim3(256), 0, st, a, f);
    });
}

using WaveSys = SysList<Sys<2, 1>, Sys<0, 1>>;
static_assert(SysAll::same_as<WaveSys>([](int kind, int nd) { return forward_wave_supported(kind, nd, 16); }), "WaveSys is forward_wave_supported");

void launch_apply_wave(int kind, const Bufs& a, int B, int T, hipStream_t st, const FwdArgs& f) {
    WaveSys::dispatch(kind, 1, [&](auto s) {
        hipLaunchKernelGGL((k_apply<decltype(s)>), dim3((B + 15) / 16, (T + 15) / 16), dim3(256), 0, st, a, f);
        hipLaunchKernelGGL(k_flip_ran, dim3((B + 255) / 256), dim3(256), 0, st, a);
    });
}

template <class S, int NA>
static void launch_select(const Bufs& a, int B, hipStream_t st, const FwdArgs& f) {
    const dim3 sgrid((B + 3) / 4);
    if (f.n_kp >= 2) {
        if (f.kp_ext) hipLaunchKernelGGL((k_select<S, NA, true, 2>), sgrid, dim3(128), 0, st, a, f);
        else hipLaunchKernelGGL((k_select<S, NA, false, 2>), sgrid, dim3(128), 0, st, a, f);
    } else {
        if (f.kp_ext) hipLaunchKernelGGL((k_select<S, NA, true, 1>), sgrid, dim3(64), 0, st, a, f);
        else hipLaunchKernelGGL((k_select<S, NA, false, 1>), sgrid, dim3(64), 0, st, a, f);
    }
}
template <int NA>
static void launch_forward_dpp(const Bufs& a, dim3 grid, hipStream_t st, const FwdArgs& f) {
    const dim3 block(64);
    if (f.limits) {
        if (f.early_stop) hipLaunchKernelGGL((k_forward_dpp<NA, true, true>), grid, block, 0, st, a, f);
        else hipLaunchKernelGGL((k_forward_dpp<NA, true, false>), grid, block, 0, st, a, f);
    } else {
        if (f.early_stop) hipLaunchKernelGGL((k_forward_dpp<NA, false, true>), grid, block, 0, st, a, f);
        else hipLaunchKernelGGL((k_forward_dpp<NA, false, false>), grid, block, 0, st, a, f);
    }
}
static void launch_forward_reg(const Bufs& a, dim3 grid, hipStream_t st, const FwdArgs& f) {
    const dim3 block(FR_WAVES * 64);
#define FR_LAUNCH_(LIM, ES)                                                                             \
    do {                                                                                                \
        if (a.kd_sym) hipLaunchKernelGGL((k_forward_reg<LIM, ES, true>), grid, block, 0, st, a, f);  \
        else hipLaunchKernelGGL((k_forward_reg<LIM, ES, false>), grid, block, 0, st, a, f);          \
    } while (0)
    if (f.limits) {
        if (f.early_stop) FR_LAUNCH_(true, true);
        else FR_LAUNCH_(true, false);
    } else {
        if (f.early_stop) FR_LAUNCH_(false, true);
        else FR_LAUNCH_(false, false);
    }
#undef FR_LAUNCH_
}
template <class S>
static void launch_forward_wave_sys(bool small, const Bufs& a, int B, hipStream_t st, const FwdArgs& f) {
    const dim3 grid(grid_x8((B + FW_IW - 1) / FW_IW)), block(FW_IW * 32);
    const dim3 rgrid(grid_x8((B + 4 * FR_WAVES - 1) / (4 * FR_WAVES)));
    const dim3 sgrid(grid_x8((B + 3) / 4));
    const auto obs_ls = [&]() { if (f.obs) launch_obs_ls(a, *f.obs, f.obs_part, B, f.obs_T, S::NX, f.n_alpha, 0, st); };
    if (f.n_alpha <= 1) {
        if (small) launch_forward_dpp<1>(a, sgrid, st, f);
        else if (f.fwd_lds) hipLaunchKernelGGL((k_forward_wg<1>), grid, block, 0, st, a, f);
        else launch_forward_reg(a, rgrid, st, f);
        obs_ls();
        launch_select<S, 1>(a, B, st, f);
    } else if (f.n_alpha <= 11) {
        if (small) launch_forward_dpp<11>(a, sgrid, st, f);
        else if (f.fwd_lds) hipLaunchKernelGGL((k_forward_wg<11>), grid, block, 0, st, a, f);
        else launch_forward_reg(a, rgrid, st, f);
        obs_ls();
        launch_select<S, 11>(a, B, st, f);
    } else {
        if (small) launch_forward_dpp<16>(a, sgrid, st, f);
        else if (f.fwd_lds) hipLaunchKernelGGL((k_forward_wg<16>), grid, block, 0, st, a, f);
        else launch_forward_reg(a, rgrid, st, f);
        obs_ls();
        launch_select<S, 16>(a, B, st, f);
    }
}
void launch_forward_wave(int kind, bool small, const Bufs& a, int B, hipStream_t st, const FwdArgs& f) {
    WaveSys::dispatch(kind, 1, [&](auto s) { launch_forward_wave_sys<decltype(s)>(small, a, B, st, f); });
}

}
```

### ilqr_planner_amd/csrc/ilqr_lanes.hpp

```cpp
#pragma once
#include <hip/hip_runtime.h>

namespace ilqr {

#define LDS_ORDER() asm volatile("" ::: "memory")
__device__ __forceinline__ void lds_barrier() { asm volatile("s_waitcnt lgkmcnt(0)\n\ts_barrier" ::: "memory"); }

template <int CTRL>
__device__ __forceinline__ double dpp_f64(double v) {
    int lo = __double2loint(v), hi = __double2hiint(v);
    lo = __builtin_amdgcn_mov_dpp(lo, CTRL, 0xf, 0xf, false);
    hi = __builtin_amdgcn_mov_dpp(hi, CTRL, 0xf, 0xf, false);
    return __hiloint2double(hi, lo);
}
template <int CTRL>
__device__ __forceinline__ double dppz_f64(double v) {
    return __builtin_amdgcn_update_dpp(0.0, v, CTRL, 0xf, 0xf, false);
}
template <int L>
__device__ __forceinline__ double dppz_bcast(double v) { return dppz_f64<0x150 + L>(v); }
template <int LO, int HI>
__device__ __forceinline__ double dpp_bcast_halves(double v, double other = 0.0) {
    const double hi = HI < 0 ? other : __builtin_amdgcn_update_dpp(0.0, v, 0x150 + (HI < 0 ? 0 : HI), 0xf, 0xc, false);
    return __builtin_amdgcn_update_dpp(hi, v, 0x150 + LO, 0xf, 0x3, false);
}
__device__ __forceinline__ double dppz_shr7(double v) { return dppz_f64<0x117>(v); }
__device__ __forceinline__ double dppz_shl7(double v) { return dppz_f64<0x107>(v); }
__device__ __forceinline__ double bperm_f64(int byte_addr, double v) {
    const int lo = __builtin_amdgcn_ds_bpermute(byte_addr, __double2loint(v));
    const int hi = __builtin_amdgcn_ds_bpermute(byte_addr, __double2hiint(v));
    return __hiloint2double(hi, lo);
}
__device__ __forceinline__ double ring_take(double v) {
    double r;
    asm volatile("v_mov_b64_e32 %0, %1" : "=v"(r) : "v"(v));
    return r;
}

__device__ __forceinline__ double quad_sum(double v) {
    v += dpp_f64<0xB1>(v);
    v += dpp_f64<0x4E>(v);
    return v;
}
__device__ __forceinline__ double oct_sum(double v) {
    v = quad_sum(v);
    v += dpp_f64<0x141>(v);
    return v;
}
__device__ __forceinline__ double oct_sum_rounded(double v) {
#pragma clang fp contract(off)
    v = v + dpp_f64<0xB1>(v);
    v = v + dpp_f64<0x4E>(v);
    v = v + dpp_f64<0x141>(v);
    return v;
}
__device__ __forceinline__ double row16_sum(double v) {
    v = oct_sum(v);
    v += dpp_f64<0x140>(v);
    return v;
}
__device__ __forceinline__ double cross_rows_sum(double v) {
    v += __shfl_xor(v, 16);
    v += __shfl_xor(v, 32);
    return v;
}
__device__ __forceinline__ double wave_sum(double v) { return cross_rows_sum(row16_sum(v)); }

}
```

### ilqr_planner_amd/csrc/ilqr_plan.hpp

```cpp
#pragma once

namespace ilqr {

constexpr int SPLIT_MIN_BATCH = 2048;
constexpr int split_first_half(int B) { return (B / 2 + 63) / 64 * 64; }


constexpr bool backward_si_supported(int kind, int nd, bool al, int m, int per_step, bool con_state_only) {
    return (kind == 0 || kind == 2) && nd == 1 && (!al || (con_state_only && per_step == 0 && m <= 4));
}
constexpr bool backward_mfma_supported(int kind, int , bool al, int m) { return kind != 2 && (!al || m <= 16); }
constexpr bool backward_rows_supported(int kind, int nd, bool al, int m) {
    return kind != 2 && !(kind == 0 && nd == 1) && (!al || m <= 16);
}
constexpr bool forward_wave_supported(int kind, int nd, int n_alpha) { return (kind == 0 || kind == 2) && nd == 1 && n_alpha <= 16; }
constexpr bool forward_lin_supported(int kind, int nd, int n_alpha) { return kind == 0 && nd == 2 && n_alpha <= 16; }
constexpr bool init_lti_supported(int kind, int nd) {
    return ((kind == 0 || kind == 1) && (nd == 1 || nd == 2)) || ((kind == 2 || kind == 3) && nd == 1);
}

constexpr bool obs_coop_supported(int kind, int nd, bool al, int m, int per_step, bool con_state_only, int n_alpha) {
    return backward_si_supported(kind, nd, al, m, per_step, con_state_only) && forward_wave_supported(kind, nd, n_alpha);
}

inline int n_alpha_of(bool line_search, double alpha_floor) {
    int n = 1;
    if (line_search) { double a = 1.0; while (a > alpha_floor && n < 64) { a *= 0.5; n++; } }
    return n;
}

constexpr int si_lanes(int launched_B, int n_simd) { return (launched_B + 3) / 4 <= n_simd ? 16 : 8; }
constexpr int SI_WG_MIN_BATCH = 256;
constexpr int SI_IO_MIN_BATCH = 256;
constexpr bool si_io_supported(bool al, int m) { return !al || m <= 1; }
constexpr int SI_PREP_MIN_BATCH = 256;

enum class SweepPin { Auto = 0, Mfma = 1, Rows = 2, SiWave = 4, SiWg = 5, SiWgIo = 6, SiWgPrep = 7 };
enum class FwdPin { Auto = 0, Wg = 1, Dpp = 2, WgLds = 3 };
enum class RerollPin { Auto = 0, Rows = 1, Dpp = 2 };

struct PlanIn {
    int kind = 0, nd = 1;
    bool al = false;
    int m = 0, per_step = 0;
    bool con_state_only = false;
    bool limits2_set = false;
    bool shared_steps = false;
    bool obstacles = false;
    bool obstacles_coop = false;
    bool uniform_R = false;
    bool off32 = true;
    bool line_search = true;
    double alpha_floor = 1e-3;
    int nb_iter = 0;
    int B = 0, n_simd = 1024;
    bool halves = false;
    int split = 1;
    bool profile = false;
    bool generic = false;
    SweepPin sweep = SweepPin::Auto;
    FwdPin forward = FwdPin::Auto;
    RerollPin reroll = RerollPin::Auto;
};

enum class Init { Lti, Generic };
enum class Sweep { SiDpp, Mfma, Rows, Generic };
enum class Forward { WaveWg, WaveDpp, Lin, Mfma, Generic };
enum class Apply {
    None,
    Wave,
    WaveLast,
    Lin,
    RerollRows,
    RerollDpp,
};
constexpr int KD_SYM_KEEP = -1;

struct RiccatiPlan {
    int n_alpha = 1;
    Init init = Init::Generic;
    bool init_al_update = false;
    Sweep sweep = Sweep::Generic;
    int si_lanes[2] = {16, 16};
    bool si_wg[2] = {false, false};
    bool si_prep[2] = {false, false};
    bool si_io[2] = {false, false};
    Forward forward = Forward::Generic;
    bool fwd_lds = false;
    Apply apply = Apply::None;
    bool al_update = false;
    bool fused = false;
    int kd_sym = 0;
    bool split = false;
    bool needs_ws = false;
    bool obs_dense = false;
};

inline RiccatiPlan plan_riccati(const PlanIn& in) {
    RiccatiPlan p;
    const int kind = in.kind, nd = in.nd;
    p.n_alpha = n_alpha_of(in.line_search, in.alpha_floor);
    if (in.obstacles && in.obstacles_coop && !in.generic && !in.limits2_set && !in.shared_steps && in.off32 &&
        obs_coop_supported(kind, nd, in.al, in.m, in.per_step, in.con_state_only, p.n_alpha)) {
        p.obs_dense = true;
        p.init = Init::Lti;
        p.init_al_update = in.al;
        p.sweep = Sweep::SiDpp;
        p.si_lanes[0] = si_lanes(in.B, in.n_simd);
        p.si_lanes[1] = si_lanes(0, in.n_simd);
        const bool dpp = in.forward == FwdPin::Dpp || (in.forward == FwdPin::Auto && (in.B + 3) / 4 <= 3 * in.n_simd / 4);
        p.forward = dpp ? Forward::WaveDpp : Forward::WaveWg;
        p.fwd_lds = in.forward == FwdPin::WgLds;
        p.apply = Apply::Wave;
        p.kd_sym = in.nb_iter == 0 ? KD_SYM_KEEP : 0;
        return p;
    }
    const bool cooperative = !in.generic && !in.limits2_set && !in.shared_steps && !in.obstacles;
    const bool coop_fwd = cooperative && p.n_alpha <= 16;

    if (cooperative && in.off32 && backward_si_supported(kind, nd, in.al, in.m, in.per_step, in.con_state_only)) p.sweep = Sweep::SiDpp;
    else if (cooperative && backward_mfma_supported(kind, nd, in.al, in.m)) {
        const bool pinned = in.sweep == SweepPin::Mfma || in.sweep == SweepPin::Rows;
        const bool rows = in.sweep == SweepPin::Rows || (!pinned && in.B > 2 * in.n_simd);
        p.sweep = rows && backward_rows_supported(kind, nd, in.al, in.m) ? Sweep::Rows : Sweep::Mfma;
    }

    if (coop_fwd && forward_wave_supported(kind, nd, p.n_alpha)) {
        const bool dpp = in.forward == FwdPin::Dpp || (in.forward == FwdPin::Auto && (in.B + 3) / 4 <= 3 * in.n_simd / 4);
        p.forward = dpp ? Forward::WaveDpp : Forward::WaveWg;
        p.fwd_lds = in.forward == FwdPin::WgLds;
    } else if (coop_fwd && forward_lin_supported(kind, nd, p.n_alpha)) {
        p.forward = Forward::Lin;
    } else if (coop_fwd) {
        p.forward = Forward::Mfma;
    }
    const bool wave = p.forward == Forward::WaveWg || p.forward == Forward::WaveDpp;
    p.fused = p.sweep == Sweep::SiDpp && wave;
    p.kd_sym = in.nb_iter == 0 ? KD_SYM_KEEP : (p.fused && in.uniform_R) ? 1 : 0;

    if (wave) p.apply = p.fused ? Apply::WaveLast : Apply::Wave;
    else if (p.forward == Forward::Lin) p.apply = Apply::Lin;
    else if (p.forward == Forward::Mfma && in.line_search) {
        const bool dpp = in.reroll == RerollPin::Dpp || (in.reroll == RerollPin::Auto && (in.B + 3) / 4 <= in.n_simd / 4);
        p.apply = dpp ? Apply::RerollDpp : Apply::RerollRows;
    }
    p.al_update = in.al && coop_fwd && !wave;

    p.init = cooperative && init_lti_supported(kind, nd) ? Init::Lti : Init::Generic;
    p.init_al_update = p.init == Init::Lti && in.al && !p.fused;

    p.split = coop_fwd && ((p.sweep == Sweep::Mfma && in.split) || in.split == 2) && !in.profile && in.halves && in.nb_iter > 0;
    p.needs_ws = p.sweep == Sweep::Generic && in.nb_iter > 0;
    const int b0 = p.split ? split_first_half(in.B) : in.B;
    p.si_lanes[0] = si_lanes(b0, in.n_simd);
    p.si_lanes[1] = si_lanes(in.B - b0, in.n_simd);
    const int launched[2] = {b0, in.B - b0};
    for (int h = 0; h < 2; h++) {
        const bool io_pin = in.sweep == SweepPin::SiWgIo || in.sweep == SweepPin::SiWgPrep;
        const bool wg_pin = in.sweep == SweepPin::SiWg || io_pin;
        p.si_wg[h] = p.sweep == Sweep::SiDpp && p.si_lanes[h] == 16 && (wg_pin || (in.sweep != SweepPin::SiWave && launched[h] >= SI_WG_MIN_BATCH));
        p.si_io[h] = p.si_wg[h] && si_io_supported(in.al, in.m) &&
                     (io_pin || (in.sweep != SweepPin::SiWg && !p.split && launched[h] >= SI_IO_MIN_BATCH));
        p.si_prep[h] = p.si_io[h] && (in.sweep == SweepPin::SiWgPrep || (in.sweep != SweepPin::SiWgIo && launched[h] >= SI_PREP_MIN_BATCH));
    }
    return p;
}

}
```

### include/ilqr_hip.h

```cpp
#ifndef ILQR_HIP_H
#define ILQR_HIP_H

#include <stddef.h>

#ifdef __cplusplus
extern "C" {
#endif

#define ILQR_MAX_SEG 24
#define ILQR_MAX_KP 8
#define ILQR_MAX_NX 15
#define ILQR_MAX_NU 8
#define ILQR_MAX_NF 15
#define ILQR_MAX_NQ 13

#define ILQR_SYS_POS_ORN 0
#define ILQR_SYS_POS_ORN_TIME 1
#define ILQR_SYS_JOINT 2
#define ILQR_SYS_JOINT_TIME 3

#define ILQR_STATUS_OK 0
#define ILQR_STATUS_NONFINITE 1
#define ILQR_STATUS_ALPHA_FLOOR 2
#define ILQR_STATUS_SWEEP_IO 4

typedef struct ilqr_ctx ilqr_ctx;
typedef struct ilqr_problem ilqr_problem;

typedef struct {
    int kind;
    int nb_deriv;
    int dof;
    int horizon;
    double dt;
    double R_diag[ILQR_MAX_NU];
    int limits_set;
    double penalty;
    double state_max[ILQR_MAX_NX + 1], state_min[ILQR_MAX_NX + 1];
    int limit_weight[ILQR_MAX_NX + 1];
    int n_seg;
    int seg_joint[ILQR_MAX_SEG];
    double seg_xyz[ILQR_MAX_SEG][3];
    double seg_R[ILQR_MAX_SEG][9];
    double seg_axis[ILQR_MAX_SEG][3];
    int n_kp;
    int kp_timestep[ILQR_MAX_KP];
    double kp_Q[ILQR_MAX_KP][ILQR_MAX_NQ * ILQR_MAX_NQ];
    int kp_dist[ILQR_MAX_KP];
    double kp_pos_radius[ILQR_MAX_KP];
    double kp_orn_thresh[ILQR_MAX_KP][3];
    int kp_has_frame[ILQR_MAX_KP];
    double kp_frame_R[ILQR_MAX_KP][9];
    double kp_frame_p[ILQR_MAX_KP][3];
    int kp_has_Ru[ILQR_MAX_KP];
    double kp_Ru[ILQR_MAX_KP][ILQR_MAX_NU];
    int kp_joint[ILQR_MAX_KP];
    int limit_multiplicity;
    int is_sequence;
    int limits2_set;
    double penalty2;
    double state_max2[ILQR_MAX_NX + 1];
    double state_min2[ILQR_MAX_NX + 1];
    int limit_weight2[ILQR_MAX_NX + 1];
    int limit_multiplicity2;
    double reg;
    double alpha_floor;
    double stop_tol;
} ilqr_problem_desc;

typedef struct { int n_x, n_u, n_f, n_Q; } ilqr_dims;
int ilqr_dims_of(const ilqr_problem_desc* desc, ilqr_dims* out);
void ilqr_desc_defaults(ilqr_problem_desc* desc);

int ilqr_chain_from_urdf(const char* urdf_text, const char* base_frame, const char* tip_frame, const double* tool_rpy,
                         const double* tool_xyz, ilqr_problem_desc* desc, double* lower, double* upper);
const char* ilqr_urdf_last_error(void);

int ilqr_ctx_create(int device_id, ilqr_ctx** out);
void ilqr_ctx_destroy(ilqr_ctx* ctx);
const char* ilqr_last_error(const ilqr_ctx* ctx);
int ilqr_ctx_set_stream(ilqr_ctx* ctx, void* hip_stream);
int ilqr_ctx_synchronize(ilqr_ctx* ctx);
int ilqr_ctx_set_split(ilqr_ctx* ctx, int on);
#define ILQR_XC_AUTO 0
#define ILQR_XC_SWEEP_MFMA 1
#define ILQR_XC_SWEEP_ROWS 2
#define ILQR_XC_SWEEP_SI_WAVE 4
#define ILQR_XC_SWEEP_SI_WG 5
#define ILQR_XC_SWEEP_SI_WG_IO 6
#define ILQR_XC_SWEEP_SI_WG_PREP 7
#define ILQR_XC_FWD_WG 1
#define ILQR_XC_FWD_DPP 2
#define ILQR_XC_FWD_WG_LDS 3
#define ILQR_XC_REROLL_ROWS 1
#define ILQR_XC_REROLL_DPP 2
int ilqr_ctx_set_crosscheck(ilqr_ctx* ctx, int generic_kernels, int cp_lane_solve, int cp_general, int sweep, int forward, int reroll);
const char* ilqr_version(void);

int ilqr_problem_create(ilqr_ctx* ctx, const ilqr_problem_desc* desc, int batch, ilqr_problem** out);
void ilqr_problem_destroy(ilqr_problem* p);

int ilqr_problem_set_init_state(ilqr_problem* p, const double* q0, const double* dq0);
int ilqr_problem_set_keypoint_targets(ilqr_problem* p, int kp_index, const double* target);
int ilqr_problem_set_controls(ilqr_problem* p, const double* U0);
int ilqr_problem_set_constraints(ilqr_problem* p, int m, int per_step, const double* A, const double* b, const double* lambda0);
int ilqr_problem_reset_multipliers(ilqr_problem* p);
int ilqr_problem_set_init_state_dev(ilqr_problem* p, const double* q0, const double* dq0);
int ilqr_problem_set_keypoint_targets_dev(ilqr_problem* p, int kp_index, const double* target);
int ilqr_problem_set_controls_dev(ilqr_problem* p, const double* U0);

int ilqr_solve_recursive(ilqr_problem* p, int nb_iter, int line_search, int early_stop);
int ilqr_solve_al(ilqr_problem* p, int nb_iter, int lag_update_step, double penalty, double scaling_factor,
                  int line_search, int early_stop);
int ilqr_solve_batch_cp(ilqr_problem* p, const double* psi, int Kw, int nb_iter, int early_stop);
int ilqr_solve_batch(ilqr_problem* p, int nb_iter, int early_stop);

int ilqr_problem_get_X(ilqr_problem* p, double* X);
int ilqr_problem_get_fX(ilqr_problem* p, double* fX);
int ilqr_problem_get_U(ilqr_problem* p, double* U);
int ilqr_problem_get_K(ilqr_problem* p, double* K);
int ilqr_problem_get_d(ilqr_problem* p, double* d);
int ilqr_problem_get_cost(ilqr_problem* p, double* cost);
int ilqr_problem_get_alpha(ilqr_problem* p, double* alpha);
int ilqr_problem_get_iters(ilqr_problem* p, int* iters);
int ilqr_problem_get_status(ilqr_problem* p, int* status);
int ilqr_problem_get_lambda(ilqr_problem* p, double* lambda);
int ilqr_problem_get_trace(ilqr_problem* p, double* cost_trace, double* alpha_trace, int nb_iter);
int ilqr_problem_get_X_dev(ilqr_problem* p, double* X);
int ilqr_problem_get_U_dev(ilqr_problem* p, double* U);
int ilqr_problem_get_cost_dev(ilqr_problem* p, double* cost);

int ilqr_problem_warm_start(ilqr_problem* p, int shift);
int ilqr_problem_track(ilqr_problem* p, int k, const double* x_meas, int with_feedforward, double* u_out);
int ilqr_problem_track_dev(ilqr_problem* p, int k, const double* x_meas, int with_feedforward, double* u_out);
int ilqr_problem_gains(ilqr_problem* p);
int ilqr_problem_gains_al(ilqr_problem* p, double penalty);
int ilqr_problem_closed_loop(ilqr_problem* p, int n_samples, const double* x0, const double* w, int with_feedforward, double* cost, double* X,
                             double* U);
int ilqr_problem_closed_loop_dev(ilqr_problem* p, int n_samples, const double* x0, const double* w, int with_feedforward, double* cost, double* X,
                                 double* U);
#define ILQR_CL_STATS 5
typedef struct {
    unsigned long long seed;
    unsigned int instance_offset, sample_offset;
    double sigma_w[ILQR_MAX_NX], sigma_x0[ILQR_MAX_NX];
} ilqr_noise;
int ilqr_problem_closed_loop_noise(ilqr_problem* p, int n_samples, const ilqr_noise* noise, const double* x0, int with_feedforward, double* cost,
                                   double* stats, double* X, double* U, double* w_out);
int ilqr_problem_closed_loop_noise_dev(ilqr_problem* p, int n_samples, const ilqr_noise* noise, const double* x0, int with_feedforward, double* cost,
                                       double* stats, double* X, double* U, double* w_out);
#define ILQR_KP_ERR 5
#define ILQR_KP_ERR_POS 0
#define ILQR_KP_ERR_ORN 1
#define ILQR_KP_ERR_VEL 2
#define ILQR_KP_ERR_ANGVEL 3
#define ILQR_KP_ERR_TIME 4
#define ILQR_KP_STATS 12
#define ILQR_CL_OUTCOME 4
typedef struct {
    double kp_tol[ILQR_MAX_KP][ILQR_KP_ERR];
    double lim_tol;
} ilqr_cl_tol;
typedef struct {
    double* kp_err;
    double* kp_stats;
    double* lim_cost;
    double* outcome;
} ilqr_cl_report;
int ilqr_problem_closed_loop_report(ilqr_problem* p, int n_samples, const ilqr_noise* noise, const double* x0, const double* w,
                                    int with_feedforward, const ilqr_cl_tol* tol, double* cost, double* stats, const ilqr_cl_report* out);
int ilqr_problem_closed_loop_report_dev(ilqr_problem* p, int n_samples, const ilqr_noise* noise, const double* x0, const double* w,
                                        int with_feedforward, const ilqr_cl_tol* tol, double* cost, double* stats, const ilqr_cl_report* out);

#define ILQR_CL_COV_KP ILQR_KP_ERR
typedef struct {
    double* Sigma;
    double* kp_Sigma;
    double* kp_var;
    double* u_var;
    double* lim_z;
} ilqr_cl_cov;
int ilqr_problem_closed_loop_cov(ilqr_problem* p, const double* sigma_w, const double* sigma_x0, const ilqr_cl_cov* out);
int ilqr_problem_closed_loop_cov_dev(ilqr_problem* p, const double* sigma_w, const double* sigma_x0, const ilqr_cl_cov* out);

#define ILQR_CL_CON_STATS 6
#define ILQR_CL_OUTCOME_CON 5
typedef struct {
    double* con_max;
    double* con_steps;
    double* con_stats;
    double* outcome_con;
} ilqr_cl_con;
int ilqr_problem_closed_loop_report_con(ilqr_problem* p, int n_samples, const ilqr_noise* noise, const double* x0, const double* w,
                                        int with_feedforward, const ilqr_cl_tol* tol, double* cost, double* stats, const ilqr_cl_report* out,
                                        double con_tol, const ilqr_cl_con* con);
int ilqr_problem_closed_loop_report_con_dev(ilqr_problem* p, int n_samples, const ilqr_noise* noise, const double* x0, const double* w,
                                            int with_feedforward, const ilqr_cl_tol* tol, double* cost, double* stats, const ilqr_cl_report* out,
                                            double con_tol, const ilqr_cl_con* con);
typedef struct {
    double* con_var;
    double* con_z;
} ilqr_cl_cov_con;
int ilqr_problem_closed_loop_cov_con(ilqr_problem* p, const double* sigma_w, const double* sigma_x0, const ilqr_cl_cov* out,
                                     const ilqr_cl_cov_con* con);
int ilqr_problem_closed_loop_cov_con_dev(ilqr_problem* p, const double* sigma_w, const double* sigma_x0, const ilqr_cl_cov* out,
                                         const ilqr_cl_cov_con* con);

#define ILQR_ADOPT_STATE 1
#define ILQR_ADOPT_TARGETS 2
#define ILQR_ADOPT_CONTROLS0 4
#define ILQR_ADOPT_CONTROLS 8
#define ILQR_ADOPT_MULTIPLIERS 16
typedef struct {
    unsigned long long seed;
    unsigned int group_offset, member_offset;
    double sigma_u[ILQR_MAX_NU];
} ilqr_seeds;
int ilqr_problem_adopt(ilqr_problem* dst, ilqr_problem* src, const int* index, int what);
int ilqr_problem_adopt_dev(ilqr_problem* dst, ilqr_problem* src, const int* index, int what);
int ilqr_problem_spread_controls(ilqr_problem* p, int group_size, const ilqr_seeds* seeds);
int ilqr_problem_spread_controls_dev(ilqr_problem* p, int group_size, const ilqr_seeds* seeds);
int ilqr_problem_select(ilqr_problem* p, int group_size, const double* score, const int* eligible, int* winner, double* best, int* n_candidates);
int ilqr_problem_select_dev(ilqr_problem* p, int group_size, const double* score, const int* eligible, int* winner, double* best, int* n_candidates);
int ilqr_problem_get_at(ilqr_problem* p, int n, const int* index, double* X, double* U, double* cost, int* iters, int* status);
int ilqr_problem_get_at_dev(ilqr_problem* p, int n, const int* index, double* X, double* U, double* cost, int* iters, int* status);

#define ILQR_CLR_MAX_SPH 32
#define ILQR_CLR_MAX_PLANES 8
#define ILQR_CLR_STATS 4
typedef struct {
    int n_sph;
    int sph_link[ILQR_CLR_MAX_SPH];
    double sph_c[ILQR_CLR_MAX_SPH][3];
    double sph_r[ILQR_CLR_MAX_SPH];
    int n_planes;
    double plane_n[ILQR_CLR_MAX_PLANES][3];
    double plane_d[ILQR_CLR_MAX_PLANES];
} ilqr_clr_robot;
typedef struct {
    const double* obs;
    int n_sets, n_obs, traj_per_set;
    double margin;
    int stats_group;
} ilqr_clr_world;
typedef struct {
    double* clr;
// ... 57 lines not shown
```

Measured before the change: 14.94 million problem-iterations/s.

## Add warp-specialized forward rollout with loader/storer helper waves and LDS ring

Adds an IO variant of the register forward kernel in which three extra helper waves own global traffic. Two loader waves stream gain records and X/U rows into an 8-slot LDS ring, and a storer wave writes results back. The four chain waves only read and write LDS and coordinate through LDS progress flags polled with a bounded spin. The aim is to take global-memory latency and block-store barriers off the serial time-step chain. In exchange it adds flag-polling overhead and a larger workgroup, and on a poll timeout it marks the instance inactive with a SWEEP_IO status. It is enabled automatically for batches of 1024 to 4096 when the wave workgroup forward is chosen and the split is off.

New measurement: 15.30 million problem-iterations/s (median of 6 runs). 1.02x the previous value.

```diff
diff --git a/ilqr_planner_amd/capi.py b/ilqr_planner_amd/capi.py
--- a/ilqr_planner_amd/capi.py
+++ b/ilqr_planner_amd/capi.py
@@ -406,7 +406,7 @@
     def synchronize(self):
         self.check(self.L.ilqr_ctx_synchronize(self.h))
 
-    _PINS = {"sweep": {None: 0, "mfma": 1, "rows": 2, "siwave": 4, "siwg": 5, "siwgio": 6, "siwgprep": 7}, "forward": {None: 0, "wg": 1, "dpp": 2, "wglds": 3}, "reroll": {None: 0, "rows": 1, "dpp": 2}}
+    _PINS = {"sweep": {None: 0, "mfma": 1, "rows": 2, "siwave": 4, "siwg": 5, "siwgio": 6, "siwgprep": 7}, "forward": {None: 0, "wg": 1, "dpp": 2, "wglds": 3, "wgio": 4}, "reroll": {None: 0, "rows": 1, "dpp": 2}}
 
     def set_crosscheck(self, generic_kernels=False, cp_lane_solve=False, cp_general=False, sweep=None, forward=None, reroll=None):
         pins = []
diff --git a/ilqr_planner_amd/csrc/ilqr_capi.cpp b/ilqr_planner_amd/csrc/ilqr_capi.cpp
--- a/ilqr_planner_amd/csrc/ilqr_capi.cpp
+++ b/ilqr_planner_amd/csrc/ilqr_capi.cpp
@@ -162,13 +162,13 @@
 
 static_assert((int)SweepPin::Mfma == ILQR_XC_SWEEP_MFMA && (int)SweepPin::Rows == ILQR_XC_SWEEP_ROWS && (int)SweepPin::SiWave == ILQR_XC_SWEEP_SI_WAVE &&
               (int)SweepPin::SiWg == ILQR_XC_SWEEP_SI_WG && (int)SweepPin::SiWgIo == ILQR_XC_SWEEP_SI_WG_IO && (int)SweepPin::SiWgPrep == ILQR_XC_SWEEP_SI_WG_PREP && (int)FwdPin::Wg == ILQR_XC_FWD_WG &&
-              (int)FwdPin::Dpp == ILQR_XC_FWD_DPP && (int)FwdPin::WgLds == ILQR_XC_FWD_WG_LDS && (int)RerollPin::Rows == ILQR_XC_REROLL_ROWS && (int)RerollPin::Dpp == ILQR_XC_REROLL_DPP,
+              (int)FwdPin::Dpp == ILQR_XC_FWD_DPP && (int)FwdPin::WgLds == ILQR_XC_FWD_WG_LDS && (int)FwdPin::WgIo == ILQR_XC_FWD_WG_IO && (int)RerollPin::Rows == ILQR_XC_REROLL_ROWS && (int)RerollPin::Dpp == ILQR_XC_REROLL_DPP,
               "variant pins of ilqr_plan.hpp and include/ilqr_hip.h");
 
 extern "C" int ilqr_ctx_set_crosscheck(ilqr_ctx* c, int generic_kernels, int cp_lane_solve, int cp_general, int sweep, int forward, int reroll) {
     if (!c) return 1;
     if (sweep < 0 || sweep > 7 || sweep == 3) return fail(c, "ilqr_ctx_set_crosscheck: sweep must be ILQR_XC_AUTO, ILQR_XC_SWEEP_MFMA, ILQR_XC_SWEEP_ROWS, ILQR_XC_SWEEP_SI_WAVE, ILQR_XC_SWEEP_SI_WG, ILQR_XC_SWEEP_SI_WG_IO or ILQR_XC_SWEEP_SI_WG_PREP");
-    if (forward < 0 || forward > 3) return fail(c, "ilqr_ctx_set_crosscheck: forward must be ILQR_XC_AUTO, ILQR_XC_FWD_WG, ILQR_XC_FWD_DPP or ILQR_XC_FWD_WG_LDS");
+    if (forward < 0 || forward > 4) return fail(c, "ilqr_ctx_set_crosscheck: forward must be ILQR_XC_AUTO, ILQR_XC_FWD_WG, ILQR_XC_FWD_DPP, ILQR_XC_FWD_WG_LDS or ILQR_XC_FWD_WG_IO");
     if (reroll < 0 || reroll > 2) return fail(c, "ilqr_ctx_set_crosscheck: reroll must be ILQR_XC_AUTO, ILQR_XC_REROLL_ROWS or ILQR_XC_REROLL_DPP");
     c->xc_sweep = (SweepPin)sweep;
     c->xc_forward = (FwdPin)forward;
@@ -687,6 +687,7 @@
     f.n_kp_all = p->desc.n_kp;
     f.fused = pl.fused ? 1 : 0;
     f.fwd_lds = pl.fwd_lds ? 1 : 0;
+    f.fwd_io = pl.fwd_io ? 1 : 0;
     f.limits = p->desc.limits_set ? 1 : 0;
     for (int k = 0; k < p->desc.n_kp; k++) f.kp_ext |= p->desc.kp_dist[k] | p->desc.kp_has_frame[k] | p->desc.kp_has_Ru[k] | p->desc.kp_joint[k];
     return f;
diff --git a/ilqr_planner_amd/csrc/ilqr_fwd_io_plan.hpp b/ilqr_planner_amd/csrc/ilqr_fwd_io_plan.hpp
--- /dev/null
+++ b/ilqr_planner_amd/csrc/ilqr_fwd_io_plan.hpp
@@ -0,0 +1,20 @@
+#pragma once
+
+namespace ilqr {
+
+constexpr int FIO_RING = 8;
+constexpr int FIO_GROUP = 4;
+static_assert(FIO_RING > FIO_GROUP, "the loaders must be able to fill the group ahead of the one the slowest chain wave is in");
+static_assert((FIO_RING & (FIO_RING - 1)) == 0 && FIO_RING % FIO_GROUP == 0, "slot = step & (FIO_RING - 1); a group never wraps inside the ring");
+
+constexpr int fio_slot(int n) { return n & (FIO_RING - 1); }
+constexpr int fio_min(int a, int b) { return a < b ? a : b; }
+
+constexpr int fio_need_loaded_g(int k0, int T1) { return fio_min(k0 + FIO_GROUP + 1, T1); }
+constexpr int fio_need_loaded_v(int k0, int T1) { return fio_min(k0 + FIO_GROUP, T1); }
+constexpr int fio_need_stored(int k0) { return k0 + FIO_GROUP - FIO_RING; }
+
+constexpr int fio_need_produced_load(int n) { return n + 1 - FIO_RING; }
+constexpr int fio_need_produced_store(int n) { return n + 1; }
+
+}
diff --git a/ilqr_planner_amd/csrc/ilqr_kernels.hpp b/ilqr_planner_amd/csrc/ilqr_kernels.hpp
--- a/ilqr_planner_amd/csrc/ilqr_kernels.hpp
+++ b/ilqr_planner_amd/csrc/ilqr_kernels.hpp
@@ -62,6 +62,7 @@
     int limits;
     int fused;
     int fwd_lds;
+    int fwd_io;
     const ObsArgs* obs;
     double* obs_part;
     int obs_T;
diff --git a/ilqr_planner_amd/csrc/ilqr_kernels_dpp.hip b/ilqr_planner_amd/csrc/ilqr_kernels_dpp.hip
--- a/ilqr_planner_amd/csrc/ilqr_kernels_dpp.hip
+++ b/ilqr_planner_amd/csrc/ilqr_kernels_dpp.hip
@@ -91,10 +91,6 @@
     return oct_sum_rounded(p) - b;
 }
 
-__device__ __forceinline__ unsigned lds_addr(const void* p) { return (unsigned)(size_t)(const __attribute__((address_space(3))) void*)p; }
-typedef __attribute__((address_space(3))) int lds_int;
-__device__ __forceinline__ int flag_read(const int* p) { LDS_ORDER(); const int v = *(const lds_int*)p; LDS_ORDER(); return v; }
-__device__ __forceinline__ void flag_write(int* p, int v) { LDS_ORDER(); *(lds_int*)p = v; LDS_ORDER(); }
 __device__ __forceinline__ int wait_consumed(int seen, unsigned addr, int need);
 __device__ __forceinline__ double ldg(const double* base, unsigned byte_off) { return *reinterpret_cast<const double*>(reinterpret_cast<const char*>(base) + byte_off); }
 __device__ __forceinline__ void stg(double* base, unsigned byte_off, double v) { *reinterpret_cast<double*>(reinterpret_cast<char*>(base) + byte_off) = v; }
@@ -109,27 +105,7 @@
 constexpr int SW_PRING = 8;
 constexpr int SW_PENT = 6;
 namespace {
-__device__ __forceinline__ int wait_consumed(int seen, unsigned addr, int need) {
-    int v = seen, cons, cnt;
-    asm volatile(
-        "s_mov_b32 %[cnt], 0\n"
-        "1:\n\t"
-        "v_readfirstlane_b32 %[cons], %[v]\n\t"
-        "s_cmp_ge_i32 %[cons], %[need]\n\t"
-        "s_cbranch_scc1 2f\n\t"
-        "s_cmp_ge_u32 %[cnt], %[lim]\n\t"
-        "s_cbranch_scc1 2f\n\t"
-        "s_sleep 1\n\t"
-        "ds_read_b32 %[v], %[addr]\n\t"
-        "s_add_u32 %[cnt], %[cnt], 1\n\t"
-        "s_waitcnt lgkmcnt(0)\n\t"
-        "s_branch 1b\n"
-        "2:"
-        : [v] "+v"(v), [cons] "=&s"(cons), [cnt] "=&s"(cnt)
-        : [addr] "v"(addr), [need] "s"(need), [lim] "s"(SW_POLL_CHAIN)
-        : "memory", "scc");
-    return __builtin_amdgcn_readfirstlane(cons < need ? 1 : 0);
-}
+__device__ __forceinline__ int wait_consumed(int seen, unsigned addr, int need) { return flag_wait_ge(seen, addr, need, SW_POLL_CHAIN); }
 }
 template <int LPI, int MR, bool FUSED, bool UNIF, bool WG = false, int IO = 0>
 __global__ __launch_bounds__(WG ? (SW_WAVES + ((IO & 7) ? 1 : 0) + ((IO & 4) ? SW_PREP : 0)) * 64 : 64) void k_backward_si_dpp(Bufs a, SweepArgs sw) {
diff --git a/ilqr_planner_amd/csrc/ilqr_kernels_wave.hip b/ilqr_planner_amd/csrc/ilqr_kernels_wave.hip
--- a/ilqr_planner_amd/csrc/ilqr_kernels_wave.hip
+++ b/ilqr_planner_amd/csrc/ilqr_kernels_wave.hip
@@ -1,6 +1,7 @@
 #include <cstdlib>
 #include <cstring>
 
+#include "ilqr_fwd_io_plan.hpp"
 #include "ilqr_lanes.hpp"
 #include "ilqr_obstacle.hpp"
 #include "ilqr_plan.hpp"
@@ -331,8 +332,12 @@
 
 constexpr int FR_WAVES = 4;
 constexpr int FR_PF = 8;
-template <bool LIM, bool ES, bool SYM>
-__global__ __launch_bounds__(FR_WAVES * 64) void k_forward_reg(Bufs a, FwdArgs f) {
+constexpr int FR_HELPERS = 3;
+constexpr int FIO_DEPTH_V = 8;
+constexpr int FIO_POLL_CHAIN = 1 << 20;
+constexpr int FIO_POLL_HELPER = 1 << 18;
+template <bool LIM, bool ES, bool SYM, bool IO = false>
+__global__ __launch_bounds__((FR_WAVES + (IO ? FR_HELPERS : 0)) * 64) void k_forward_reg(Bufs a, FwdArgs f) {
 #pragma clang fp contract(off)
     constexpr int NX = 7, NU = 7, ROWP = kd_rowp(NX), PF = FR_PF, IPW = 4;
     static_assert(ROWP == 8, "record row = 7 gains + feed-forward");
@@ -340,9 +345,13 @@
     constexpr int RSD = SYM ? KD_SYM_RS : NU * ROWP;
     constexpr int NPC = IPW * RSD / 2;
     static_assert(NPC > 64 && NPC <= 128, "two pieces per lane");
-    __shared__ __attribute__((aligned(16))) double sK[FR_WAVES][2][IPW * RSD];
+    __shared__ __attribute__((aligned(16))) double sK[IO ? 1 : FR_WAVES][2][IO ? 2 : IPW * RSD];
     constexpr int NR = NX + NU, IWG = FR_WAVES * IPW, OSTR = IWG + 2, NT = FR_WAVES * 64, NOUT = PF * NR * IWG, NRND = (NOUT + NT - 1) / NT;
-    __shared__ double sOut[2][PF * NR * OSTR];
+    __shared__ double sOut[IO ? 1 : 2][IO ? 1 : PF * NR * OSTR];
+    __shared__ __attribute__((aligned(16))) double sG[IO ? FIO_RING : 1][IO ? IWG * RSD : 2];
+    __shared__ double sIn[IO ? FIO_RING : 1][IO ? (NR + 1) * OSTR : 1];
+    __shared__ double sOu[IO ? FIO_RING : 1][IO ? (NR + 1) * OSTR : 1];
+    __shared__ int sFl[IO ? FR_WAVES + 3 : 1];
     const DevDesc& d = *a.desc;
     const int wv = __builtin_amdgcn_readfirstlane((int)threadIdx.x >> 6);
     const int lane = threadIdx.x & 63, g = lane >> 4, l = lane & 15, h = l >> 3, r8 = l & 7;
@@ -354,6 +363,124 @@
         const int bi = b0 - wv * IPW + (lane & (IWG - 1));
         const bool any = (bi < B) && (a.active[bi < B ? bi : 0] != 0);
         if (__ballot(any ? 1 : 0) == 0ull) return;
+    }
+    if constexpr (IO) {
+        if (wv == 0 && lane < FR_WAVES + 3) sFl[lane] = 0;
+        if (wv >= FR_WAVES) {
+            const int wgb0 = xcd_tile() * IWG, li = lane & (IWG - 1), rq = lane >> 4;
+            const int bi = wgb0 + li;
+            const bool in = bi < B;
+            const int bbi = in ? bi : 0;
+            const bool oki = in && (a.active[bbi] != 0);
+            const int curi = a.cur[bbi];
+            __syncthreads();
+            const unsigned livem = (unsigned)__ballot((oki && lane < IWG) ? 1 : 0);
+            const int T1 = T - 1;
+            const size_t Vstep = (size_t)NX * Bp;
+            int have = 0;
+            auto wait_produced = [&](int need) -> bool {
+                if (have >= need) return true;
+                const bool want = lane < FR_WAVES && ((livem >> (lane * IPW)) & 15u) != 0u;
+                for (int spins = 0;; spins++) {
+                    const int pv = flag_read(&sFl[lane < FR_WAVES ? lane : 0]);
+                    if (__ballot((want && pv < need) ? 1 : 0) == 0ull) {
+                        int mn = 0x7fffffff;
+                        UNR for (int w = 0; w < FR_WAVES; w++) {
+                            const int pw = __builtin_amdgcn_readlane(pv, w);
+                            if (((livem >> (w * IPW)) & 15u) != 0u && pw < mn) mn = pw;
+                        }
+                        have = mn;
+                        return true;
+                    }
+                    if (spins >= FIO_POLL_HELPER) return false;
+                    __builtin_amdgcn_s_sleep(4);
+                }
+            };
+            auto give_up = [&]() {
+                if (lane < IWG && in) { a.active[bbi] = 0; atomicOr(&a.status[bbi], ILQR_STATUS_SWEEP_IO); }
+            };
+            int lrow[4];
+            UNR for (int q = 0; q < 4; q++) lrow[q] = (rq + 4 * q < NR ? rq + 4 * q : NR) * OSTR + li;
+            if (wv == FR_WAVES) {
+                constexpr int NP16 = IWG * RSD / 2, NPQ = (NP16 + 63) / 64, DG = SYM ? 8 : 6;
+                static_assert(DG * NPQ <= 63, "the loader stays within the vector-memory counter");
+                typedef double d2v __attribute__((ext_vector_type(2)));
+                const char* kb = reinterpret_cast<const char*>(a.KD + (size_t)wgb0 * RSD);
+                const size_t Kstep = (size_t)Bp * RSD * sizeof(double);
+                unsigned pc16[NPQ];
+                UNR for (int q = 0; q < NPQ; q++) pc16[q] = (unsigned)(lane + 64 * q < NP16 ? lane + 64 * q : NP16 - 1);
+                double ga[DG][NPQ], gb[DG][NPQ];
+                auto fetch = [&](int slot, int kk) {
+                    UNR for (int q = 0; q < NPQ; q++) {
+                        const d2v v = __builtin_nontemporal_load(reinterpret_cast<const d2v*>(kb + pc16[q] * 16u));
+                        ga[slot][q] = v.x; gb[slot][q] = v.y;
+                    }
+                    kb += (kk < T - 2) ? Kstep : 0;
+                };
+                UNR for (int q = 0; q < DG; q++) { fetch(q, q); __builtin_amdgcn_sched_barrier(0); }
+                for (int n0 = 0; n0 < T1; n0 += DG) {
+                    UNR for (int jj = 0; jj < DG; jj++) {
+                        const int n = n0 + jj;
+                        if (n < T1) {
+                            if (!wait_produced(fio_need_produced_load(n))) { give_up(); return; }
+                            double* im = &sG[fio_slot(n)][0];
+                            UNR for (int q = 0; q < NPQ; q++) {
+                                const double ta = ring_take(ga[jj][q]), tb = ring_take(gb[jj][q]);
+                                *reinterpret_cast<double2*>(im + 2 * pc16[q]) = make_double2(ta, tb);
+                            }
+                            flag_write(&sFl[FR_WAVES], n + 1);
+                        }
+                        __builtin_amdgcn_sched_barrier(0);
+                        fetch(jj, n + DG);
+                    }
+                }
+            } else if (wv == FR_WAVES + 1) {
+                constexpr int DV = FIO_DEPTH_V;
+                const double* pv[4];
+                UNR for (int q = 0; q < 4; q++) {
+                    const int rw = rq + 4 * q < NR ? rq + 4 * q : NR - 1;
+                    pv[q] = (rw < NX ? a.X[curi] + (size_t)rw * Bp : a.U[curi] + (size_t)(rw - NX) * Bp) + bbi;
+                }
+                double xv[DV][4];
+                auto fetch = [&](int slot, int kk) {
+                    UNR for (int q = 0; q < 4; q++) { xv[slot][q] = *pv[q]; pv[q] += (kk < T - 2) ? Vstep : 0; }
+                };
+                UNR for (int q = 0; q < DV; q++) { fetch(q, q); __builtin_amdgcn_sched_barrier(0); }
+                for (int n0 = 0; n0 < T1; n0 += DV) {
+                    UNR for (int jj = 0; jj < DV; jj++) {
+                        const int n = n0 + jj;
+                        if (n < T1) {
+                            if (!wait_produced(fio_need_produced_load(n))) { give_up(); return; }
+                            double* im = &sIn[fio_slot(n)][0];
+                            UNR for (int q = 0; q < 4; q++) im[lrow[q]] = ring_take(xv[jj][q]);
+                            flag_write(&sFl[FR_WAVES + 1], n + 1);
+                        }
+                        __builtin_amdgcn_sched_barrier(0);
+                        fetch(jj, n + DV);
+                    }
+                }
+            } else {
+                double* pd[4];
+                bool sto[4];
+                UNR for (int q = 0; q < 4; q++) {
+                    const int rw = rq + 4 * q < NR ? rq + 4 * q : NR - 1;
+                    sto[q] = oki && rq + 4 * q < NR;
+                    pd[q] = (rw < NX ? a.X[1 - curi] + (size_t)rw * Bp : a.U[1 - curi] + (size_t)(rw - NX) * Bp) + bbi;
+                }
+                for (int n = 0; n < T1; n++) {
+                    if (!wait_produced(fio_need_produced_store(n))) { give_up(); return; }
+                    LDS_ORDER();
+                    const double* im = &sOu[fio_slot(n)][0];
+                    double v[4];
+                    UNR for (int q = 0; q < 4; q++) v[q] = im[lrow[q]];
+                    flag_write(&sFl[FR_WAVES + 2], n + 1);
+                    UNR for (int q = 0; q < 4; q++) { if (sto[q]) *pd[q] = v[q]; pd[q] += Vstep; }
+                }
+            }
+            return;
+        }
+        __syncthreads();
+        if (__ballot(inst_ok ? 1 : 0) == 0ull) return;
     }
     const int bb = (b < B) ? b : 0;
     const bool row = r8 < NX;
@@ -424,16 +551,18 @@
             K[0] = v0.x; K[1] = v0.y; K[2] = v1.x; K[3] = v1.y;
         }
     };
-    UNR for (int q = 0; q < PF; q++) { fetch_g(q, q); fetch_v(q, q); __builtin_amdgcn_sched_barrier(0); }
     double Kc[4];
-    stage(0, 0);
-    LDS_ORDER();
-    pick(0, Kc);
-    stage(1, 1);
-    LDS_ORDER();
-    __builtin_amdgcn_sched_barrier(0);
-    fetch_g(0, PF);
-    fetch_g(1, PF + 1);
+    if constexpr (!IO) {
+        UNR for (int q = 0; q < PF; q++) { fetch_g(q, q); fetch_v(q, q); __builtin_amdgcn_sched_barrier(0); }
+        stage(0, 0);
+        LDS_ORDER();
+        pick(0, Kc);
+        stage(1, 1);
+        LDS_ORDER();
+        __builtin_amdgcn_sched_barrier(0);
+        fetch_g(0, PF);
+        fetch_g(1, PF + 1);
+    }
 
     double dx = 0, dun = 0, pc[4] = {0, 0, 0, 0};
     auto pair_cost = [&](double v0, double mx0, double mn0, double v1, double mx1, double mn1) -> double {
@@ -471,12 +600,20 @@
         __builtin_amdgcn_sched_barrier(0);                           \
         fetch_g((JJ + 2) % PF, k + 2 + PF);                                                                        \
         if (!CHK || k < T - 1) {                                                                                   \
-            const double vb = ring_take(vr[JJ]);                                              \
+            FR_BODY_(CHK, ring_take(vr[JJ]), sOut[ob][JJ * NR * OSTR + ow])                                        \
+        }                                                                                                          \
+        __builtin_amdgcn_sched_barrier(0);                                                                         \
+        fetch_v(JJ, k + PF);                                                                                       \
+        UNR for (int j = 0; j < 4; j++) Kc[j] = Kn[j];                                                             \
+    }
+#define FR_BODY_(CHK, VB, OUT)                                                                                     \
+        {                                                                                                          \
+            const double vb = VB;                                                             \
             const double x0 = dpp_bcast_halves<0, 4>(dx), x1 = dpp_bcast_halves<1, 5>(dx);                         \
             const double x2 = dpp_bcast_halves<2, 6>(dx), x3 = dpp_bcast_halves<3, -1>(dx, 1.0);                   \
             const double part = fma(Kc[0], x0, Kc[1] * x1) + fma(Kc[2], x2, Kc[3] * x3);                           \
             const double du = part + dpp_f64<0x128>(part);                   \
-            sOut[ob][JJ * NR * OSTR + ow] = vb + (h ? du : dx);                               \
+            OUT = vb + (h ? du : dx);                                                         \
             if (ES) {                                     \
                 const double o = dpp_f64<0xB1>(du);                                      \
                 const double pa = ev ? du : o, pb = ev ? o : du;                                                   \
@@ -493,17 +630,55 @@
                 kp_next = (kpi < n_kp) ? __builtin_amdgcn_readfirstlane(d.kp_t[kpi]) : -1;                         \
             }                                                                                                      \
             dx = fma(dt, du, dx);                                            \
-        }                                                                                                          \
-        __builtin_amdgcn_sched_barrier(0);                                                                         \
-        fetch_v(JJ, k + PF);                                                                                       \
-        UNR for (int j = 0; j < 4; j++) Kc[j] = Kn[j];                                                             \
-    }
-    for (int k0 = 0, ob = 0; k0 < T - 1; k0 += PF, ob ^= 1) {
-        UNR for (int jj = 0; jj < PF; jj++) FR_STEP_(jj, true)
-        lds_barrier();
-        block_store(ob, k0);
+        }
+    if constexpr (!IO) {
+        for (int k0 = 0, ob = 0; k0 < T - 1; k0 += PF, ob ^= 1) {
+            UNR for (int jj = 0; jj < PF; jj++) FR_STEP_(jj, true)
+            lds_barrier();
+            block_store(ob, k0);
+        }
+    } else {
+        constexpr int G = FIO_GROUP;
+        const int T1 = T - 1;
+        const unsigned fl_g = lds_addr(&sFl[FR_WAVES]), fl_v = lds_addr(&sFl[FR_WAVES + 1]), fl_s = lds_addr(&sFl[FR_WAVES + 2]);
+        const int go = (wv * IPW) * RSD;
+        auto pick_io = [&](int slot, double (&K)[4]) {
+            const double* im = &sG[slot][go];
+            if (SYM) {
+                UNR for (int j = 0; j < 4; j++) K[j] = im[ro[j]];
+            } else {
+                const double2 v0 = *reinterpret_cast<const double2*>(im + ro[0]), v1 = *reinterpret_cast<const double2*>(im + ro[2]);
+                K[0] = v0.x; K[1] = v0.y; K[2] = v1.x; K[3] = v1.y;
+            }
+        };
+        int gave = flag_wait_ge(flag_read(&sFl[FR_WAVES]), fl_g, fio_need_loaded_g(0, T1), FIO_POLL_CHAIN);
+        LDS_ORDER();
+        pick_io(0, Kc);
+        for (int k0 = 0; k0 < T1; k0 += G) {
+            const int seen_g = flag_read(&sFl[FR_WAVES]), seen_v = flag_read(&sFl[FR_WAVES + 1]), seen_s = flag_read(&sFl[FR_WAVES + 2]);
+            gave |= flag_wait_ge(seen_g, fl_g, __builtin_amdgcn_readfirstlane(fio_need_loaded_g(k0, T1)), FIO_POLL_CHAIN);
+            gave |= flag_wait_ge(seen_v, fl_v, __builtin_amdgcn_readfirstlane(fio_need_loaded_v(k0, T1)), FIO_POLL_CHAIN);
+            gave |= flag_wait_ge(seen_s, fl_s, __builtin_amdgcn_readfirstlane(fio_need_stored(k0)), FIO_POLL_CHAIN);
+            if (gave) break;
+            const int s0 = fio_slot(k0);
+            UNR for (int jj = 0; jj < G; jj++) {
+                const int k = k0 + jj;
+                double Kn[4];
+                pick_io(jj + 1 < G ? s0 + jj + 1 : fio_slot(k0 + G), Kn);
+                if (k < T1) {
+                    FR_BODY_(true, sIn[s0 + jj][ow], sOu[s0 + jj][ow])
+                    flag_write(&sFl[wv], k + 1);
+                }
+                UNR for (int j = 0; j < 4; j++) Kc[j] = Kn[j];
+            }
+        }
+        if (gave) {
+            if (inst_ok && l == 0) { a.active[bb] = 0; atomicOr(&a.status[bb], ILQR_STATUS_SWEEP_IO); }
+            return;
+        }
     }
 #undef FR_STEP_
+#undef FR_BODY_
     {
         if (sx) a.X[1 - cur][((size_t)(T - 1) * NX + r) * Bp + bb] = xT + dx;
         if (LIM && __ballot((seg_bad(xT) & sx) ? 1 : 0) != 0ull) limits_all(xT);
@@ -807,11 +982,14 @@
     }
 }
 static void launch_forward_reg(const Bufs& a, dim3 grid, hipStream_t st, const FwdArgs& f) {
-    const dim3 block(FR_WAVES * 64);
-#define FR_LAUNCH_(LIM, ES)                                                                             \
-    do {                                                                                                \
-        if (a.kd_sym) hipLaunchKernelGGL((k_forward_reg<LIM, ES, true>), grid, block, 0, st, a, f);  \
-        else hipLaunchKernelGGL((k_forward_reg<LIM, ES, false>), grid, block, 0, st, a, f);          \
+    const dim3 block(FR_WAVES * 64), ioblock((FR_WAVES + FR_HELPERS) * 64);
+#define FR_LAUNCH_(LIM, ES)                                                                                                     \
+    do {                                                                                                                        \
+        if (f.fwd_io) {                                                                                                         \
+            if (a.kd_sym) hipLaunchKernelGGL((k_forward_reg<LIM, ES, true, true>), grid, ioblock, 0, st, a, f);                 \
+            else hipLaunchKernelGGL((k_forward_reg<LIM, ES, false, true>), grid, ioblock, 0, st, a, f);                         \
+        } else if (a.kd_sym) hipLaunchKernelGGL((k_forward_reg<LIM, ES, true>), grid, block, 0, st, a, f);                      \
+        else hipLaunchKernelGGL((k_forward_reg<LIM, ES, false>), grid, block, 0, st, a, f);                                     \
     } while (0)
     if (f.limits) {
         if (f.early_stop) FR_LAUNCH_(true, true);
diff --git a/ilqr_planner_amd/csrc/ilqr_lanes.hpp b/ilqr_planner_amd/csrc/ilqr_lanes.hpp
--- a/ilqr_planner_amd/csrc/ilqr_lanes.hpp
+++ b/ilqr_planner_amd/csrc/ilqr_lanes.hpp
@@ -5,6 +5,32 @@
 
 #define LDS_ORDER() asm volatile("" ::: "memory")
 __device__ __forceinline__ void lds_barrier() { asm volatile("s_waitcnt lgkmcnt(0)\n\ts_barrier" ::: "memory"); }
+
+__device__ __forceinline__ unsigned lds_addr(const void* p) { return (unsigned)(size_t)(const __attribute__((address_space(3))) void*)p; }
+typedef __attribute__((address_space(3))) int lds_int;
+__device__ __forceinline__ int flag_read(const int* p) { LDS_ORDER(); const int v = *(const lds_int*)p; LDS_ORDER(); return v; }
+__device__ __forceinline__ void flag_write(int* p, int v) { LDS_ORDER(); *(lds_int*)p = v; LDS_ORDER(); }
+__device__ __forceinline__ int flag_wait_ge(int seen, unsigned addr, int need, int polls) {
+    int v = seen, cons, cnt;
+    asm volatile(
+        "s_mov_b32 %[cnt], 0\n"
+        "1:\n\t"
+        "v_readfirstlane_b32 %[cons], %[v]\n\t"
+        "s_cmp_ge_i32 %[cons], %[need]\n\t"
+        "s_cbranch_scc1 2f\n\t"
+        "s_cmp_ge_u32 %[cnt], %[lim]\n\t"
+        "s_cbranch_scc1 2f\n\t"
+        "s_sleep 1\n\t"
+        "ds_read_b32 %[v], %[addr]\n\t"
+        "s_add_u32 %[cnt], %[cnt], 1\n\t"
+        "s_waitcnt lgkmcnt(0)\n\t"
+        "s_branch 1b\n"
+        "2:"
+        : [v] "+v"(v), [cons] "=&s"(cons), [cnt] "=&s"(cnt)
+        : [addr] "v"(addr), [need] "s"(need), [lim] "s"(polls)
+        : "memory", "scc");
+    return __builtin_amdgcn_readfirstlane(cons < need ? 1 : 0);
+}
 
 template <int CTRL>
 __device__ __forceinline__ double dpp_f64(double v) {
diff --git a/ilqr_planner_amd/csrc/ilqr_plan.hpp b/ilqr_planner_amd/csrc/ilqr_plan.hpp
--- a/ilqr_planner_amd/csrc/ilqr_plan.hpp
+++ b/ilqr_planner_amd/csrc/ilqr_plan.hpp
@@ -35,8 +35,12 @@
 constexpr bool si_io_supported(bool al, int m) { return !al || m <= 1; }
 constexpr int SI_PREP_MIN_BATCH = 256;
 
+constexpr int FWD_IO_MIN_BATCH = 1024;
+constexpr int FWD_IO_MAX_BATCH = 4096;
+constexpr bool fwd_io_auto(int launched_B) { return launched_B >= FWD_IO_MIN_BATCH && launched_B <= FWD_IO_MAX_BATCH; }
+
 enum class SweepPin { Auto = 0, Mfma = 1, Rows = 2, SiWave = 4, SiWg = 5, SiWgIo = 6, SiWgPrep = 7 };
-enum class FwdPin { Auto = 0, Wg = 1, Dpp = 2, WgLds = 3 };
+enum class FwdPin { Auto = 0, Wg = 1, Dpp = 2, WgLds = 3, WgIo = 4 };
 enum class RerollPin { Auto = 0, Rows = 1, Dpp = 2 };
 
 struct PlanIn {
@@ -87,6 +91,7 @@
     bool si_io[2] = {false, false};
     Forward forward = Forward::Generic;
     bool fwd_lds = false;
+    bool fwd_io = false;
     Apply apply = Apply::None;
     bool al_update = false;
     bool fused = false;
@@ -111,6 +116,7 @@
         const bool dpp = in.forward == FwdPin::Dpp || (in.forward == FwdPin::Auto && (in.B + 3) / 4 <= 3 * in.n_simd / 4);
         p.forward = dpp ? Forward::WaveDpp : Forward::WaveWg;
         p.fwd_lds = in.forward == FwdPin::WgLds;
+        p.fwd_io = in.forward == FwdPin::WgIo;
         p.apply = Apply::Wave;
         p.kd_sym = in.nb_iter == 0 ? KD_SYM_KEEP : 0;
         return p;
@@ -151,6 +157,7 @@
 
     p.split = coop_fwd && ((p.sweep == Sweep::Mfma && in.split) || in.split == 2) && !in.profile && in.halves && in.nb_iter > 0;
     p.needs_ws = p.sweep == Sweep::Generic && in.nb_iter > 0;
+    p.fwd_io = p.forward == Forward::WaveWg && !p.fwd_lds && (in.forward == FwdPin::WgIo || (in.forward == FwdPin::Auto && !p.split && fwd_io_auto(in.B)));
     const int b0 = p.split ? split_first_half(in.B) : in.B;
     p.si_lanes[0] = si_lanes(b0, in.n_simd);
     p.si_lanes[1] = si_lanes(in.B - b0, in.n_simd);
diff --git a/include/ilqr_hip.h b/include/ilqr_hip.h
--- a/include/ilqr_hip.h
+++ b/include/ilqr_hip.h
@@ -92,6 +92,7 @@
 #define ILQR_XC_FWD_WG 1
 #define ILQR_XC_FWD_DPP 2
 #define ILQR_XC_FWD_WG_LDS 3
+#define ILQR_XC_FWD_WG_IO 4
 #define ILQR_XC_REROLL_ROWS 1
 #define ILQR_XC_REROLL_DPP 2
 int ilqr_ctx_set_crosscheck(ilqr_ctx* ctx, int generic_kernels, int cp_lane_solve, int cp_general, int sweep, int forward, int reroll);
```
